# blasif/cocons

Measured on AMD Instinct MI355X. Metric: -2loglik evals/sec (dense cov_rns + Cholesky/solve/log-det, fp64) at n=10000, higher is better.
Workload: dtype f64

## Files before the change

cocons_amd/csrc/api.hip:

```cpp
#include <hip/hip_runtime.h>
#include <limits.h>
#include <math.h>
#include <stdarg.h>
#include <stdint.h>
#include <stdio.h>
#include <stdlib.h>
#include <string.h>
#include <unistd.h>
#include <time.h>
#include <dlfcn.h>
#include <rccl/rccl.h>

#include <algorithm>
#include <limits>
#include <memory>
#include <mutex>
#include <string>
#include <thread>
#include <vector>

#include "kernels.h"
#include "../../include/cocons_hip_diag.h"
#include "matern_device.hpp"

// ... 139 lines not shown
    bool fix = true;
    for (int i = 1; i < p; ++i)
        if (theta[TH_SMOOTH * p + i] != 0) fix = false;
    if (fix && smooth_limits[0] == smooth_limits[1]) {
        double v = smooth_limits[0];
        m.nu_fixed = v;
        m.smooth_kind = SMOOTH_ZERO;
        if (std::fabs(v - 0.5) < 1e-6) m.mode = MODE_HALF;
        else if (std::fabs(v - 1.5) < 1e-6) m.mode = MODE_THREEHALF;
        else if (std::fabs(v - 2.5) < 1e-6) m.mode = MODE_FIVEHALF;
        else m.mode = MODE_GEOM;
    } else {
        m.mode = MODE_GEOM;
        m.smooth_kind = SMOOTH_LOGISTIC_SQRT;
    }
    return m;
}

static LocArgs loc_args(int n, int p, const double *X, const double *locs, double *out, size_t stride, const ThetaVecs &tv,
                        int smooth_kind, const double *smooth_limits)
{
    LocArgs la;
    la.n = n; la.p = p;
    la.X = X; la.ldx = n;
    la.locs = locs; la.ldl = n;
    la.out = out; la.stride = stride;
    la.smooth_kind = smooth_kind;
    la.smooth_min = smooth_limits[0]; la.smooth_max = smooth_limits[1];
    la.th = tv;
    return la;
}

static inline int round_up(int v, int m) { return (v + m - 1) / m * m; }

struct RcclApi {
    void *h;
    ncclResult_t (*GetUniqueId)(ncclUniqueId *);
    ncclResult_t (*CommInitRank)(ncclComm_t *, int, ncclUniqueId, int);
    ncclResult_t (*CommInitAll)(ncclComm_t *, int, const int *);
    ncclResult_t (*CommDestroy)(ncclComm_t);
    ncclResult_t (*Broadcast)(const void *, void *, size_t, ncclDataType_t, int, ncclComm_t, hipStream_t);
    ncclResult_t (*AllReduce)(const void *, void *, size_t, ncclDataType_t, ncclRedOp_t, ncclComm_t, hipStream_t);
    ncclResult_t (*AllGather)(const void *, void *, size_t, ncclDataType_t, ncclComm_t, hipStream_t);
    ncclResult_t (*GroupStart)();
    ncclResult_t (*GroupEnd)();
    const char *(*GetErrorString)(ncclResult_t);
    ncclResult_t (*CommCount)(const ncclComm_t, int *);
    ncclResult_t (*CommUserRank)(const ncclComm_t, int *);
    ncclResult_t (*CommCuDevice)(const ncclComm_t, int *);
    ncclResult_t (*CommAbort)(ncclComm_t);
    ncclResult_t (*Send)(const void *, size_t, ncclDataType_t, int, ncclComm_t, hipStream_t);
    ncclResult_t (*Recv)(void *, size_t, ncclDataType_t, int, ncclComm_t, hipStream_t);
    ncclResult_t (*CommSplit)(ncclComm_t, int, int, ncclComm_t *, void *);
};

static RcclApi *rccl_api()
{
    static RcclApi api;
    static int state = 0;
    if (state == 0) {
        state = -1;
        std::vector<std::string> names;
        {
            Dl_info di;
            if (dladdr((void *)&hipGetDeviceCount, &di) && di.dli_fname) {
                std::string dir(di.dli_fname);
                size_t slash = dir.rfind('/');
                if (slash != std::string::npos) {
                    dir.resize(slash + 1);
                    names.push_back(dir + "librccl.so.1");
                    names.push_back(dir + "librccl.so");
                }
            }
        }
        names.push_back("librccl.so.1");
        names.push_back("librccl.so");
        names.push_back("/opt/rocm/lib/librccl.so.1");
        void *h = nullptr;
        for (const std::string &nm : names)
            if ((h = dlopen(nm.c_str(), RTLD_NOW | RTLD_LOCAL))) break;
        if (!h) { g_err = std::string("cannot load RCCL: ") + dlerror(); return nullptr; }
        api.h = h;
#define RSYM(field, name) *(void **)(&api.field) = dlsym(h, name); if (!api.field) { g_err = "RCCL symbol missing: " name; return nullptr; }
        RSYM(GetUniqueId, "ncclGetUniqueId")
        RSYM(CommInitRank, "ncclCommInitRank")
        RSYM(CommInitAll, "ncclCommInitAll")
        RSYM(CommDestroy, "ncclCommDestroy")
        RSYM(Broadcast, "ncclBroadcast")
        RSYM(AllReduce, "ncclAllReduce")
        RSYM(AllGather, "ncclAllGather")
        RSYM(GroupStart, "ncclGroupStart")
        RSYM(GroupEnd, "ncclGroupEnd")
        RSYM(GetErrorString, "ncclGetErrorString")
        RSYM(CommCount, "ncclCommCount")
        RSYM(CommUserRank, "ncclCommUserRank")
        RSYM(CommCuDevice, "ncclCommCuDevice")
        RSYM(CommAbort, "ncclCommAbort")
        RSYM(Send, "ncclSend")
        RSYM(Recv, "ncclRecv")
#undef RSYM
        *(void **)(&api.CommSplit) = dlsym(h, "ncclCommSplit");
        state = 1;
    }
    return state == 1 ? &api : nullptr;
}

static void rccl_comm_destroy(ncclComm_t c)
{
    RcclApi *R = rccl_api();
    if (R && c) R->CommDestroy(c);
}

#define NCCLCHK(expr)                                                             \
    do {                                                                          \
        ncclResult_t r__ = (expr);                                                \
        if (r__ != ncclSuccess) {                                                 \
            char b__[512];                                                        \
            snprintf(b__, sizeof b__, "%s failed: %s (%s:%d)", #expr,             \
                     rccl_api() ? rccl_api()->GetErrorString(r__) : "?", __FILE__, __LINE__); \
            g_err = b__;                                                          \
            return -200 - (int)r__;                                               \
        }                                                                         \
    } while (0)

struct cocons_fit {
    int n, p, r, q, device;
    pid_t pid;
    int npad, nt;
    int rhs_cap;
    int rhs_act;
    size_t lda;
    hipStream_t stream;
    bool own_stream;
    double *dX, *dlocs, *dz, *dxb;
    double *dloc;
    double *dA;
    double *dinv;
    int *dinfo;
    double *dout;
    double *hout;
    int *hinfo, *hinfo_init = nullptr;
    double smooth_limits[2];
    size_t out_cap;
    double *dlocp, *dXp, *dlocsp, *dstoch, *dquad, *dred;
    int pred_cap;
    int rank, world, nrhs_cur;
    int nslot;
    int n_user, pad0;
    double *xbuf[2];
    size_t xbuf_bytes;
    bool xbuf_own;
    hipEvent_t ev[8];
    hipStream_t stream2;
    hipEvent_t ev_eng;
    unsigned *dflags;
    int flags_cap;
    bool engine_ok;
    bool engine_live;
    bool engine_used;
    int border_clean = -1;
    int border_pending = -1;
    bool engine_active_last;
    int engine_skip;
    int engine_fails;
    int engine_retries;
    int engine_last_abort;
    long long engine_ops;
    double *dP; size_t dP_elems;
    double *dWt; int dWt_tiles;
    double *dpart;
    unsigned *ddag; size_t ddag_words;
    void *ddag_steps; int dag_nsteps; unsigned dag_ntasks;
    int dag_key[13];
    unsigned *ddag_ftab; size_t ddag_ftab_words;
    int dag_xcd_g;
    bool dag_have_ftab;
    size_t ddag_xcnt_off;
    unsigned long long *ddag_trace; size_t dag_trace_tasks;
    size_t dag_trace_elems;
    bool dag_next;
    int engine_pair_live;
    int engine_t0;
    size_t smb_off, smb_elems;
    size_t xmb_off, xmb_elems;
    double *dmbox; size_t dmbox_elems;
    bool follow_used, follow_off;
    double enq_host_us; long long enq_calls;
    bool dag_used;
    double dag_flops; int dag_events;
    int taper_nnz;
    int *d_tci, *d_trp;
    double *d_tval;
    std::vector<int> *taper_hi;
    int *d_thi; int taper_maxband;
    int skew;
    std::vector<int> *taper_inv;
    std::vector<int> *h_trp, *h_tci;
    std::vector<double> *h_tval;
    cocons_fit *taper_twin;
    std::vector<int> *twin_perm;
    float sim_ms[3];
    int coll_kind;
    int coll_rank, coll_world;
    ncclComm_t comm;
    bool comm_own;
    cocons_bcast_fn cb_bcast;
    cocons_allreduce_fn cb_allreduce;
    cocons_allgather_fn cb_allgather;
    struct ShardState *shard;
    void *cb_user;
    hipStream_t cstream;
    hipStream_t cstream_l;
    ncclComm_t comm_l;
    bool comm_l_own;
    double *dcoll;
    double upd_flops;
    std::vector<double> *h_locs, *h_X, *h_z, *h_xb;
    std::vector<cocons_fit *> *slots;
    bool sorted;
    cocons_fit *unsorted;
    std::recursive_mutex *op_mu;
    struct KrigeState *krige;
};

struct KrigeState {
    DevBuf<double> L;
    DevBuf<double> Q;
    DevBuf<double> w;
    DevBuf<double> loc;
    DevBuf<double> C;
    DevBuf<double> Xp, lp, locp;
    DevBuf<double> st, qd;
    std::vector<double> theta;
    int rows = 0;
    long long bytes = 0;
};

static void shard_state_free(struct ShardState *S);

static std::mutex g_reg_mutex;
static std::vector<cocons_fit *> g_registry;
static void registry_add(cocons_fit *f) { std::lock_guard<std::mutex> lk(g_reg_mutex); g_registry.push_back(f); }
static void registry_remove(cocons_fit *f)
{
    std::lock_guard<std::mutex> lk(g_reg_mutex);
    g_registry.erase(std::remove(g_registry.begin(), g_registry.end(), f), g_registry.end());
}

static int fit_check(cocons_fit *f)
{
    if (!f) return fail(-1, "null fit handle");
    if (f->pid != getpid())
        return fail(-2, "fit handle was created in another process (fork); create it in the worker");
    hipError_t e = hipSetDevice(f->device);
    if (e != hipSuccess) return fail(-3, "hipSetDevice: %s", hipGetErrorString(e));
    return 0;
}

#define FIT_ENTER(f)                                                   \
    if (int rc__ = fit_check(f)) return rc__;                          \
    std::lock_guard<std::recursive_mutex> op_guard__(*(f)->op_mu)

static int fit_alloc_matrix(cocons_fit *f, int rhs_rows)
{
    int cap = round_up(rhs_rows > 0 ? rhs_rows : 1, TILE);
    f->rhs_act = cap;
    f->border_clean = -1; f->border_pending = -1;
    if (f->dA && cap <= f->rhs_cap) return 0;
    if (f->dA) { HIPCHK(hipFree(f->dA)); f->dA = nullptr; }
    f->rhs_cap = cap;
    f->lda = (size_t)(f->skew > 0 ? f->skew * TILE : f->npad) + cap;
    HIPCHK(hipMalloc(&f->dA, f->lda * (size_t)f->npad * sizeof(double)));
    HIPCHK(hipMemsetAsync(f->dA, 0, f->lda * (size_t)f->npad * sizeof(double), f->stream));
    HIPCHK(hipStreamSynchronize(f->stream));
    return 0;
}

extern "C" void cocons_fit_destroy(cocons_fit *f)
{
    if (!f) return;
    registry_remove(f);
    if (f->op_mu) { f->op_mu->lock(); f->op_mu->unlock(); }
    if (f->pid == getpid()) {
        hipSetDevice(f->device);
        if (f->stream) hipStreamSynchronize(f->stream);
        if (f->stream2) hipStreamSynchronize(f->stream2);
        hipFree(f->dX); hipFree(f->dlocs); hipFree(f->dz); hipFree(f->dxb); hipFree(f->dloc);
        hipFree(f->dA); hipFree(f->dinv); hipFree(f->dinfo);
        hipFree(f->dlocp); hipFree(f->dXp); hipFree(f->dlocsp); hipFree(f->dstoch); hipFree(f->dquad); hipFree(f->dred);
        if (f->xbuf_own) { hipFree(f->xbuf[0]); hipFree(f->xbuf[1]); }
        hipHostFree(f->hinfo);
        for (auto &e : f->ev) if (e) hipEventDestroy(e);
        if (f->ev_eng) hipEventDestroy(f->ev_eng);
        hipFree(f->dflags);
        if (f->dmbox) hipFree(f->dmbox);
        hipFree(f->dP); hipFree(f->dWt); hipFree(f->ddag); hipFree(f->ddag_steps); hipFree(f->ddag_trace); hipFree(f->dpart);
        hipFree(f->ddag_ftab);
        hipFree(f->d_tci); hipFree(f->d_trp); hipFree(f->d_tval); hipFree(f->d_thi);
        if (f->cstream_l && f->cstream_l != f->cstream) { hipStreamSynchronize(f->cstream_l); hipStreamDestroy(f->cstream_l); }
        if (f->cstream) { hipStreamSynchronize(f->cstream); hipStreamDestroy(f->cstream); }
        shard_state_free(f->shard);
        hipFree(f->dcoll);
        if (f->comm_l && f->comm_l_own) rccl_comm_destroy(f->comm_l);
        if (f->comm && f->comm_own) rccl_comm_destroy(f->comm);
        if (f->slots) { for (auto c : *f->slots) cocons_fit_destroy(c); delete f->slots; f->slots = nullptr; }
        if (f->unsorted) { cocons_fit_destroy(f->unsorted); f->unsorted = nullptr; }
        if (f->taper_twin) { cocons_fit_destroy(f->taper_twin); f->taper_twin = nullptr; }
        delete f->krige; f->krige = nullptr;
        if (f->stream2) hipStreamDestroy(f->stream2);
        if (f->own_stream && f->stream) hipStreamDestroy(f->stream);
    }
    delete f->h_locs; delete f->h_X; delete f->h_z; delete f->h_xb;
    delete f->taper_hi; delete f->taper_inv;
    delete f->h_trp; delete f->h_tci; delete f->h_tval; delete f->twin_perm;
    delete f->op_mu;
    delete f;
}

static int engine_warm(cocons_fit *f);

static cocons_fit *fit_create_impl(int n, int p, int r, int q, const double *locs,
                                   const double *X, const double *z, const double *x_betas,
                                   const double *smooth_limits, int device, bool allow_sort, bool defer_matrix = false,
                                   bool want_engine = true, bool return_locked = false)
{
    if (n <= 0 || p <= 0 || p > COCONS_P_MAX || r < 0 || q < 0 || !locs || !X || !smooth_limits ||
        (r > 0 && !z) || (q > 0 && !x_betas)) {
        fail(-1, "cocons_fit_create: bad argument");
        return nullptr;
    }
    cocons_fit *f = new cocons_fit();
    memset(f, 0, sizeof *f);
    f->op_mu = new std::recursive_mutex();
    f->n = n; f->p = p; f->r = r; f->q = q;
    f->device = device < 0 ? 0 : device;
    f->pid = getpid();
    f->npad = round_up(n, TILE);
    f->nt = f->npad / TILE;
    f->smooth_limits[0] = smooth_limits[0];
    f->smooth_limits[1] = smooth_limits[1];
    f->world = 1;
#define CK(expr)                                                                  \
    do {                                                                          \
        hipError_t e__ = (expr);                                                  \
        if (e__ != hipSuccess) {                                                  \
            fail(-100, "cocons_fit_create: %s", hipGetErrorString(e__));          \
            cocons_fit_destroy(f);                                                \
            return nullptr;                                                       \
        }                                                                         \
    } while (0)
    CK(hipSetDevice(f->device));
    CK(hipStreamCreateWithFlags(&f->stream, hipStreamNonBlocking));
    f->own_stream = true;
    std::vector<int> perm(n);
    for (int i = 0; i < n; ++i) perm[i] = i;
    {
        const char *e = getenv("COCONS_SPATIAL_SORT");
        if (allow_sort && (e ? atoi(e) : 1) && n > 64) {
            double lo[2] = {locs[0], locs[n]}, hi[2] = {locs[0], locs[n]};
            for (int i = 0; i < n; ++i)
                for (int d = 0; d < 2; ++d) {
                    double v = locs[i + (size_t)d * n];
                    if (v < lo[d]) lo[d] = v;
                    if (v > hi[d]) hi[d] = v;
                }
            std::vector<unsigned long long> key(n);
            bool finite = true;
            for (int i = 0; i < n && finite; ++i) {
                unsigned q[2];
                for (int d = 0; d < 2; ++d) {
                    double span = hi[d] - lo[d];
                    double t = span > 0 ? (locs[i + (size_t)d * n] - lo[d]) / span : 0.0;
                    if (!(t >= 0.0 && t <= 1.0)) { finite = false; t = 0; }
                    q[d] = (unsigned)(t * 65535.0);
                }
                unsigned long long k = 0;
                for (int b = 0; b < 16; ++b)
                    k |= ((unsigned long long)((q[0] >> b) & 1u) << (2 * b)) | ((unsigned long long)((q[1] >> b) & 1u) << (2 * b + 1));
                key[i] = (k << 32) | (unsigned)i;
            }
            if (finite) {
                std::sort(key.begin(), key.end());
                auto path = [&](auto idx) {
                    double s = 0;
                    for (int i = 0; i + 1 < n; ++i) {
                        int a = idx(i), b = idx(i + 1);
                        double dx = locs[a] - locs[b], dy = locs[a + (size_t)n] - locs[b + (size_t)n];
                        s += std::sqrt(dx * dx + dy * dy);
                    }
                    return s;
                };
                double p_in = path([&](int i) { return i; });
                double p_mo = path([&](int i) { return (int)(key[i] & 0xffffffffu); });
                if (p_mo < 0.8 * p_in)
                    for (int i = 0; i < n; ++i) perm[i] = (int)(key[i] & 0xffffffffu);
            }
        }
    }
    f->h_locs = new std::vector<double>(locs, locs + (size_t)2 * n);
    f->h_X = new std::vector<double>(X, X + (size_t)n * p);
    f->h_z = new std::vector<double>();
    if (r > 0) f->h_z->assign(z, z + (size_t)n * r);
    f->h_xb = new std::vector<double>();
    if (q > 0) f->h_xb->assign(x_betas, x_betas + (size_t)n * q);
    f->sorted = false;
    for (int i = 0; i < n; ++i)
        if (perm[i] != i) { f->sorted = true; break; }
    f->n_user = n;
    {
        const char *e = getenv("COCONS_FRONT_PAD");
        f->pad0 = (allow_sort && (e ? atoi(e) : 1)) ? f->npad - n : 0;
        const char *e2 = getenv("COCONS_RHS_SLOTS");
        const int need = round_up(r + (q > p ? q : p) > 0 ? r + (q > p ? q : p) : 1, 16);
        f->nslot = (f->pad0 >= need && r > 0 && (e2 ? atoi(e2) : 1)) ? need : 0;
        f->pad0 -= f->nslot;
    }
    const int pad0 = f->pad0, nint = n + pad0;
    if (pad0 > 0) f->sorted = true;
    auto permute_pad = [&](const double *src, int ncol, bool zero_pad) {
        std::vector<double> out((size_t)nint * ncol);
        for (int c = 0; c < ncol; ++c) {
            for (int i = 0; i < pad0; ++i) out[(size_t)i + (size_t)c * nint] = zero_pad ? 0.0 : canon_nan(src[(size_t)perm[0] + (size_t)c * n]);
            for (int i = 0; i < n; ++i) out[(size_t)(pad0 + i) + (size_t)c * nint] = canon_nan(src[(size_t)perm[i] + (size_t)c * n]);
        }
        return out;
    };
    std::vector<double> plocs = permute_pad(locs, 2, false), pX = permute_pad(X, p, false), pz, pxb;
    if (r > 0) pz = permute_pad(z, r, true);
    if (q > 0) pxb = permute_pad(x_betas, q, true);
    locs = plocs.data(); X = pX.data();
    if (r > 0) z = pz.data();
    if (q > 0) x_betas = pxb.data();
    n = nint;
    f->n = n;
    CK(hipMalloc(&f->dX, (size_t)n * p * sizeof(double)));
    CK(hipMalloc(&f->dlocs, (size_t)n * 2 * sizeof(double)));
    CK(hipMemcpyAsync(f->dX, X, (size_t)n * p * sizeof(double), hipMemcpyHostToDevice, f->stream));
    CK(hipMemcpyAsync(f->dlocs, locs, (size_t)n * 2 * sizeof(double), hipMemcpyHostToDevice, f->stream));
    if (r > 0) {
        CK(hipMalloc(&f->dz, (size_t)n * r * sizeof(double)));
        CK(hipMemcpyAsync(f->dz, z, (size_t)n * r * sizeof(double), hipMemcpyHostToDevice, f->stream));
    }
    if (q > 0) {
        CK(hipMalloc(&f->dxb, (size_t)n * q * sizeof(double)));
        CK(hipMemcpyAsync(f->dxb, x_betas, (size_t)n * q * sizeof(double), hipMemcpyHostToDevice, f->stream));
    }
    CK(hipStreamSynchronize(f->stream));
    CK(hipMalloc(&f->dloc, (size_t)LOCP_FIELDS * f->npad * sizeof(double)));
    CK(hipMalloc(&f->dinv, 2 * 8 * 256 * sizeof(double)));
    int nr_max = r + (q > p ? q : p);
    f->out_cap = (size_t)(1 + nr_max * nr_max) * (size_t)(f->nt + 2);
    {
        double *dbase = nullptr, *hbase = nullptr;
        CK(hipMalloc(&dbase, (f->out_cap + 1) * sizeof(double)));
        CK(hipHostMalloc(&hbase, (f->out_cap + 2) * sizeof(double)));
        f->dinfo = (int *)dbase; f->dout = dbase + 1;
        f->hinfo = (int *)hbase; f->hout = hbase + 1;
        f->hinfo_init = (int *)(hbase + 1 + f->out_cap);
        f->hinfo_init[0] = 0x7f7f7f7f; f->hinfo_init[1] = 0;
    }
    for (auto &e : f->ev) CK(hipEventCreate(&e));
    f->engine_ok = want_engine;
// ... 258 lines not shown
    make_theta_vecs(theta, f->p, tv, true);
    ModeSel ms = select_mode(theta, f->p, f->smooth_limits, 0);
    launch_loc_params(loc_args(f->n, f->p, f->dX, f->dlocs, f->dloc, f->npad, tv, ms.smooth_kind, f->smooth_limits), f->stream);
    if (f->d_thi) launch_band_zero(f->dA, f->lda, f->d_thi, f->nt, f->taper_maxband, f->stream, f->skew);
    else HIPCHK(hipMemsetAsync(f->dA, 0, f->lda * (size_t)f->npad * sizeof(double), f->stream));
    launch_taper(ms.mode, false, f->n, f->taper_nnz, f->d_tci, f->d_trp, f->dloc, f->npad, f->dloc, f->npad,
                 ms.nu_fixed, nullptr, f->stream, f->d_tval, f->dA, f->lda, 0, f->skew, f->npad);
    launch_pad_identity(f->dA, f->lda, f->n, f->npad, f->stream, f->skew);
    return 0;
}

static int no_taper(cocons_fit *f, const char *who)
{
    if (f->taper_nnz > 0) return fail(-1, "%s: not available on a taper fit (cocons_neg2loglik_dense is)", who);
    return 0;
}

static void assemble_rhs(cocons_fit *f, const double *mean, bool use_trend, const double *xb, int nxb,
                         int col0, int col1, bool zero_rest = true, bool slots = false)
{
    if (slots) { zero_rest = false; col1 = f->n; }
    RhsArgs ra;
    memset(&ra, 0, sizeof ra);
    ra.n = f->n; ra.p = f->p; ra.X = f->dX; ra.ldx = f->n;
    ra.use_trend = use_trend ? 1 : 0;
    if (use_trend) for (int i = 0; i < f->p; ++i) ra.mean[i] = canon_nan(mean[i]);
    ra.src = f->dz; ra.lds = f->n;
    ra.out = f->dA; ra.ld = f->lda;
    ra.skew = f->skew; ra.npad = f->npad;
    ra.row0 = slots ? f->n : f->npad; ra.nrows = f->r;
    ra.nrows_zero = (nxb > 0 || !zero_rest) ? 0 : f->rhs_act - f->r;
    ra.col0 = col0; ra.ncols_out = col1;
    launch_rhs_rows(ra, f->stream);
    if (nxb > 0) {
        ra.use_trend = 0;
        ra.src = xb; ra.lds = f->n;
        ra.row0 = (slots ? f->n : f->npad) + f->r; ra.nrows = nxb;
        ra.nrows_zero = zero_rest ? f->rhs_act - f->r - nxb : 0;
        launch_rhs_rows(ra, f->stream);
    }
}

static void residual_row(cocons_fit *f, const double *mean, int z_col, double *out, size_t ld, int row0, int nrows_zero,
                         int ncols)
{
    RhsArgs ra;
    memset(&ra, 0, sizeof ra);
    ra.n = f->n; ra.p = f->p; ra.X = f->dX; ra.ldx = f->n; ra.use_trend = 1;
    for (int i = 0; i < f->p; ++i) ra.mean[i] = canon_nan(mean[i]);
    ra.src = f->dz + (size_t)z_col * f->n; ra.lds = f->n;
    ra.out = out; ra.ld = ld; ra.row0 = row0; ra.nrows = 1; ra.nrows_zero = nrows_zero;
    ra.col0 = 0; ra.ncols_out = ncols;
    ra.skew = f->skew; ra.npad = f->npad;
    launch_rhs_rows(ra, f->stream);
}

static void clear_border(cocons_fit *f)
{
    RhsArgs ra;
    memset(&ra, 0, sizeof ra);
    ra.n = f->n; ra.p = f->p; ra.X = f->dX; ra.ldx = f->n; ra.src = f->dX; ra.lds = f->n;
    ra.out = f->dA; ra.ld = f->lda; ra.row0 = f->npad; ra.nrows = 0; ra.nrows_zero = f->rhs_act;
    ra.col0 = 0; ra.ncols_out = f->npad;
    ra.skew = f->skew; ra.npad = f->npad;
    launch_rhs_rows(ra, f->stream);
}

static std::vector<double> host_trend(const cocons_fit *f, const double *mean)
{
    const int n = f->n;
    std::vector<double> tr(n, 0.0);
    for (int j = 0; j < f->p; ++j)
        for (int i = 0; i < n; ++i) tr[i] += (*f->h_X)[(size_t)i + (size_t)j * n] * mean[j];
    return tr;
}

struct FactorView {
    double *A;
    size_t lda;
    int nt, mt;
    const int *hi = nullptr;
    int skew = 0;
    int trim = 0;
    bool dag_ok = false;
};

static FactorView main_view(cocons_fit *f)
{
    FactorView v;
    v.A = f->dA; v.lda = f->lda; v.nt = f->nt; v.mt = f->nt + f->rhs_act / TILE;
    v.hi = (f->taper_hi && !f->taper_hi->empty()) ? f->taper_hi->data() : nullptr;
    v.skew = f->skew;
    return v;
}

static int band_hi(const FactorView &v, int k)
{
    if (!v.hi) return -1;
    int h = v.hi[k];
    if (k + 1 < v.nt && v.hi[k + 1] > h) h = v.hi[k + 1];
    const int need = k + 4 < v.nt ? k + 4 : v.nt;
    if (h < need) h = need;
    return h < v.nt ? h : v.nt;
}

static bool follow_on(cocons_fit *f);
static void potrf_solve(cocons_fit *f, double *A, size_t lda, int tile, int r0, int r1, double *q, hipStream_t s, int br, int er)
{
    if (follow_on(f) && ((size_t)tile + 1) * ENGINE_MBOX_DOUBLES <= f->smb_off) {
        f->follow_used = true;
        launch_potrf_follow(A, lda, tile * TILE, r0, r1, q, f->dinfo,
                            f->dmbox + (size_t)tile * ENGINE_MBOX_DOUBLES, (unsigned *)(f->dinfo + 1), s, br, er);
        return;
    }
    launch_potrf_tile(A, lda, tile * TILE, q, f->dinfo, s);
    launch_trsm_tile(A, lda, tile * TILE, r0, r1, q, s, nullptr, nullptr, br, er);
}

static void panel_ops(cocons_fit *f, const FactorView &v, int k, hipStream_t s)
{
    const int nt = v.nt, mt = v.mt;
    double *A = v.A;
    const size_t lda = v.lda;
    double *q0 = f->dinv, *q1 = f->dinv + 8 * 256;
    const int hb = band_hi(v, k);
    const int br = hb >= 0 ? hb * TILE : -1, er = nt * TILE;
    const int r1 = mt * TILE - 64 * v.trim;
    potrf_solve(f, A, lda, k, (k + 1) * TILE, r1, q0, s, br, er);
    if (k + 1 < nt) {
        launch_update(A, lda, k * TILE, TILE, k + 1, mt, k + 1, k + 2, true, s, nullptr, -1, nullptr, nullptr, nullptr, hb, nt,
                      0, v.trim);
        potrf_solve(f, A, lda, k + 1, (k + 2) * TILE, r1, q1, s, br, er);
    }
}

struct Tunables {
    int engine = 1;
    int upd_dynamic = 1;
    int dag = 1;
    int dag_lead = 1600, dag_lead2 = 600, dag_lead3 = 1800;
    int dag_min_tiles = 2000;
    int dag_split = 1;
    int dag_xcd = 1;
    int dag_order = 1, dag_bw = 16, dag_bh = 16;
    int dag_xcd_min_quota = 128;
    int dag_xcc_quota = -1;
    int engine_block0 = 1;
    int engine_pair = 1;
    int panel_fused = 1;
    int panel_follow = 1;
    int panel_split = 32;
    int panel_diag = 1;
    int potrf_follow = 1;
    int dag_trace = 0;
    int gate_sabotage = 0;
    int host_delay_us = 0, host_delay_tile = -1, engine_in_wait_ms = 0;
    bool init = false;
};
static Tunables &tun()
{
    static Tunables t;
    if (!t.init) {
        auto rd = [](const char *name, int &v) { const char *e = getenv(name); if (e) v = atoi(e); };
        rd("COCONS_ENGINE", t.engine);
        rd("COCONS_UPD_DYNAMIC", t.upd_dynamic);
        rd("COCONS_DAG", t.dag);
        rd("COCONS_DAG_LEAD", t.dag_lead);
        rd("COCONS_DAG_LEAD2", t.dag_lead2);
        rd("COCONS_DAG_LEAD3", t.dag_lead3);
        rd("COCONS_DAG_MIN_TILES", t.dag_min_tiles);
        rd("COCONS_DAG_SPLIT", t.dag_split);
        rd("COCONS_DAG_XCC_QUOTA", t.dag_xcc_quota);
        rd("COCONS_DAG_XCD", t.dag_xcd);
        rd("COCONS_DAG_ORDER", t.dag_order);
        rd("COCONS_DAG_BW", t.dag_bw);
        rd("COCONS_DAG_BH", t.dag_bh);
        rd("COCONS_ENGINE_PAIR", t.engine_pair);
        rd("COCONS_ENGINE_BLOCK0", t.engine_block0);
        rd("COCONS_PANEL_FUSED", t.panel_fused);
        rd("COCONS_POTRF_FOLLOW", t.potrf_follow);
        rd("COCONS_PANEL_FOLLOW", t.panel_follow);
        rd("COCONS_PANEL_DIAG", t.panel_diag);
        rd("COCONS_PANEL_SPLIT", t.panel_split);
        rd("COCONS_DEBUG_HOST_DELAY_US", t.host_delay_us);
        rd("COCONS_DEBUG_HOST_DELAY_TILE", t.host_delay_tile);
        t.init = true;
    }
    return t;
}

static bool follow_on(cocons_fit *f)
{
    return tun().potrf_follow != 0 && !f->follow_off && f->dmbox != nullptr &&
           f->smb_off >= ((size_t)f->nt + 2) * ENGINE_MBOX_DOUBLES;
}

extern "C" int cocons_debug_tune(const char *name, int value)
{
    if (!name) return fail(-1, "cocons_debug_tune: null name");
    Tunables &t = tun();
    std::string k(name);
    if (k == "engine") t.engine = value;
    else if (k == "upd_dynamic") t.upd_dynamic = value;
    else if (k == "dag") t.dag = value;
    else if (k == "dag_lead") t.dag_lead = value;
    else if (k == "dag_lead2") t.dag_lead2 = value;
    else if (k == "dag_lead3") t.dag_lead3 = value;
    else if (k == "dag_min_tiles") t.dag_min_tiles = value;
    else if (k == "dag_split") t.dag_split = value;
    else if (k == "dag_xcc_quota") t.dag_xcc_quota = value;
    else if (k == "dag_xcd") t.dag_xcd = value;
    else if (k == "dag_order") t.dag_order = value;
    else if (k == "dag_xcd_min_quota") t.dag_xcd_min_quota = value;
    else if (k == "dag_bw") t.dag_bw = value < 1 ? 1 : value;
    else if (k == "dag_bh") t.dag_bh = value < 1 ? 1 : value;
    else if (k == "dag_trace") t.dag_trace = value;
    else if (k == "engine_pair") t.engine_pair = value;
    else if (k == "engine_block0") t.engine_block0 = value;
    else if (k == "panel_fused") t.panel_fused = value;
    else if (k == "potrf_follow") t.potrf_follow = value;
    else if (k == "panel_follow") t.panel_follow = value;
    else if (k == "panel_diag") t.panel_diag = value;
    else if (k == "panel_split") t.panel_split = value;
    else if (k == "gate_sabotage") t.gate_sabotage = value;
    else if (k == "host_delay_us") t.host_delay_us = value;
    else if (k == "host_delay_tile") t.host_delay_tile = value;
    else if (k == "engine_in_wait_ms") t.engine_in_wait_ms = value;
    else if (k == "upd_waves") set_update_waves(value);
    else if (k == "w8_max_tiles") set_update_w8_max_tiles(value);
    else if (k == "c_wt") set_update_c_wt(value);
    else return fail(-1, "cocons_debug_tune: unknown switch %s", name);
    return 0;
}

static int device_cus()
{
    int dev = 0, cus = 256;
    (void)hipGetDevice(&dev);
    (void)hipDeviceGetAttribute(&cus, hipDeviceAttributeMultiprocessorCount, dev);
    return cus;
}

static int dag_xcc_quota()
{
    if (tun().dag_xcc_quota >= 0) return tun().dag_xcc_quota;
    static int derived = -1;
    if (derived < 0) {
        int dev = 0, cus = 256;
        (void)hipGetDevice(&dev);
        (void)hipDeviceGetAttribute(&cus, hipDeviceAttributeMultiprocessorCount, dev);
        const int xcds = 8;
        const int cpx = cus % xcds == 0 ? cus / xcds : 32;
        derived = (cpx - 1) * 7 - 9;
        if (derived < 8) derived = 8;
    }
    return derived;
}

static bool engine_enabled() { return tun().engine != 0; }

static void timed_update(cocons_fit *f, const FactorView &v, int k, int kw, int t0, int t1, hipStream_t s,
                         std::vector<hipEvent_t> *ev_upd, unsigned *sig, int sig_tile, unsigned *queue = nullptr,
                         int skip_tiles = 0)
{
    const int mt = v.mt;
    if (t1 <= t0) return;
    const int hb = band_hi(v, k);
    if (hb >= 0 && hb < t1) t1 = hb;
    if (t1 <= t0) return;
    unsigned *abort_word = sig ? (unsigned *)(f->dinfo + 1) : nullptr;
    hipEvent_t a = nullptr, b = nullptr;
    if (ev_upd) {
        hipEventCreate(&a); hipEventCreate(&b);
        hipEventRecord(a, s);
    }
    const int kskip = (k == 0 && !v.hi) ? (f->pad0 / 16) * 16 : 0;
    launch_update(v.A, v.lda, k * TILE + kskip, kw * TILE - kskip, t0, mt, t0, t1, true, s, sig, sig_tile, nullptr,
                  abort_word, queue, hb, v.nt, 0, v.trim, skip_tiles > 0 ? 2 * t0 : 0, skip_tiles > 0 ? 2 * (t0 + skip_tiles) : 0);
    if (ev_upd) {
        hipEventRecord(b, s);
        ev_upd->push_back(a); ev_upd->push_back(b);
    }
}

static void count_update_flops(cocons_fit *f, int kw, int t0)
{
    double m = (double)f->n_user - ((double)t0 * TILE - (double)f->pad0);
    if (m > (double)f->n_user) m = (double)f->n_user;
    if (m < 0) m = 0;
    const double K = (double)kw * TILE - (t0 == kw ? (double)f->pad0 : 0.0);
    f->upd_flops += K * m * (m + 1.0) + 2.0 * K * (double)f->nrhs_cur * m;
}

static bool engine_wanted(cocons_fit *f, const FactorView &v)
{
    return engine_enabled() && f->engine_ok && f->stream2 != nullptr && f->engine_skip == 0 && v.nt > 4;
}

static int flags_reset(cocons_fit *f, int nt)
{
    if (f->flags_cap < nt) {
        if (f->stream2) HIPCHK(hipStreamSynchronize(f->stream2));
        if (f->dflags) { HIPCHK(hipFree(f->dflags)); f->dflags = nullptr; }
        f->flags_cap = round_up(nt + 8, 64);
        HIPCHK(hipMalloc(&f->dflags, (4 * (size_t)f->flags_cap + 64) * sizeof(unsigned)));
    }
    HIPCHK(hipMemsetAsync(f->dflags, 0, (4 * (size_t)f->flags_cap + 64) * sizeof(unsigned), f->stream));
    return 0;
}

static int mbox_reset(cocons_fit *f, int nt, bool engine_schedule = true)
{
    const size_t tiles = ((size_t)nt + 2) * ENGINE_MBOX_DOUBLES;
    const bool panel = tun().panel_follow && tun().panel_fused && tun().engine_pair;
    const size_t smb = panel && tun().panel_diag ? ((size_t)nt / 2 + 2) * PANEL_SMBOX_DOUBLES : 0;
    const size_t xmb = panel && tun().panel_split ? (2 * ((size_t)nt + 2) + 4) * PANEL_XMBOX_DOUBLES : 0;
    const size_t need = tiles + smb + xmb;
    if (f->dmbox_elems < need) {
        HIPCHK(hipStreamSynchronize(f->stream));
        if (f->stream2) HIPCHK(hipStreamSynchronize(f->stream2));
        if (f->dmbox) { HIPCHK(hipFree(f->dmbox)); f->dmbox = nullptr; f->dmbox_elems = 0; }
        HIPCHK(hipMalloc(&f->dmbox, need * sizeof(double)));
        f->dmbox_elems = need;
    }
    f->smb_off = tiles; f->smb_elems = smb;
    f->xmb_off = tiles + smb; f->xmb_elems = xmb;
    HIPCHK(hipMemsetAsync(f->dmbox, 0xff, (engine_schedule ? need : tiles) * sizeof(double), f->stream));
    return 0;
}

static unsigned *tile_queue(cocons_fit *f, int k)
{
    const int dyn = tun().upd_dynamic;
    return dyn ? f->dflags + 3 * (size_t)f->flags_cap + 64 + k / 2 : nullptr;
}

static int engine_warm(cocons_fit *f)
{
    if (!engine_enabled() || f->nt <= 4 || !f->engine_ok) { f->engine_ok = f->engine_ok && f->stream2 != nullptr; return 0; }
    if (!f->stream2) HIPCHK(hipStreamCreateWithFlags(&f->stream2, hipStreamNonBlocking));
    if (int rc = flags_reset(f, f->nt)) return rc;
    HIPCHK(hipStreamSynchronize(f->stream));
    {
        std::vector<hipStream_t> losers;
        int ok = 0;
        for (int attempt = 0; attempt < 8; ++attempt) {
            ok = streams_run_concurrently(f->stream2, f->stream, f->dflags + 3 * (size_t)f->flags_cap + 8);
            if (ok != 0) break;
            losers.push_back(f->stream2);
            f->stream2 = nullptr;
            if (hipStreamCreateWithFlags(&f->stream2, hipStreamNonBlocking) != hipSuccess) { ok = -1; break; }
        }
        unsigned *words = f->dflags + 3 * (size_t)f->flags_cap + 8;
        for (int round = 0; ok == 1 && round < 8; ++round) {
            std::vector<cocons_fit *> others;
            {
                std::lock_guard<std::mutex> lk(g_reg_mutex);
                for (size_t i = g_registry.size(); i-- > 0 && others.size() < 4;) {
                    cocons_fit *o = g_registry[i];
                    if (o == f || o->pid != f->pid || o->device != f->device || !o->own_stream || !o->stream || !o->stream2 ||
                        !o->engine_ok || !o->op_mu->try_lock())
                        continue;
                    if (hipStreamQuery(o->stream) == hipSuccess && hipStreamQuery(o->stream2) == hipSuccess) others.push_back(o);
                    else o->op_mu->unlock();
                }
            }
            (void)hipGetLastError();
            int clash = 0;
            for (cocons_fit *o : others) {
                int a = streams_run_concurrently(f->stream2, o->stream, words);
                if (a < 0) { ok = -1; break; }
                if (a == 0) { clash = 1; break; }
                if (f->own_stream) {
                    int b = streams_run_concurrently(o->stream2, f->stream, words);
                    if (b < 0) { ok = -1; break; }
                    if (b == 0) { clash = 2; break; }
                }
            }
            for (cocons_fit *o : others) o->op_mu->unlock();
            if (ok != 1 || clash == 0) break;
            hipStream_t &mine = clash == 1 ? f->stream2 : f->stream;
            losers.push_back(mine);
            mine = nullptr;
            if (hipStreamCreateWithFlags(&mine, hipStreamNonBlocking) != hipSuccess) { ok = -1; break; }
            int again = streams_run_concurrently(f->stream2, f->stream, words);
            if (again < 0) { ok = -1; break; }
            if (again == 0) {
                hipStream_t &other = clash == 1 ? f->stream2 : f->stream;
                (void)other;
                bool fixed = false;
                for (int t2 = 0; t2 < 4 && !fixed; ++t2) {
                    losers.push_back(mine);
                    mine = nullptr;
                    if (hipStreamCreateWithFlags(&mine, hipStreamNonBlocking) != hipSuccess) { ok = -1; break; }
                    const int r2 = streams_run_concurrently(f->stream2, f->stream, words);
                    if (r2 < 0) { ok = -1; break; }
                    fixed = r2 == 1;
                }
                if (ok != 1) break;
                if (!fixed) { ok = 0; break; }
            }
        }
        for (hipStream_t l : losers) hipStreamDestroy(l);
        if (ok < 0) { (void)hipGetLastError(); return fail(-100, "engine_warm: stream self-test failed"); }
        if (ok == 0) { f->engine_ok = false; return 0; }
        HIPCHK(hipMemsetAsync(f->dflags, 0, (4 * (size_t)f->flags_cap + 64) * sizeof(unsigned), f->stream));
        HIPCHK(hipStreamSynchronize(f->stream));
    }
    launch_potrf_engine(nullptr, 0, 0, 0, f->dinv, f->dinfo, f->dflags, f->dflags, f->dflags, (unsigned *)(f->dinfo + 1),
                        f->dflags + 3 * (size_t)f->flags_cap, f->stream2);
    if (tun().dag)
        launch_potrf_engine(nullptr, 0, 0, 0, f->dinv, f->dinfo, f->dflags, f->dflags, f->dflags, (unsigned *)(f->dinfo + 1),
                            f->dflags + 3 * (size_t)f->flags_cap, f->stream2, f->dinv, f->dinv, 0);
    HIPCHK(hipGetLastError());
    if (f->stream2) HIPCHK(hipStreamSynchronize(f->stream2));
    return 0;
}

static bool dag_wanted(cocons_fit *f, const FactorView &v)
{
    return tun().dag != 0 && v.dag_ok && !v.hi && !v.skew && v.nt > 4 && f->world == 1;
}

static int dag_prepare(cocons_fit *f, const FactorView &v)
{
    const size_t elems = v.lda * (size_t)f->npad;
    if (f->dP_elems != elems) {
        HIPCHK(hipStreamSynchronize(f->stream));
        if (f->stream2) HIPCHK(hipStreamSynchronize(f->stream2));
        if (f->dP) { HIPCHK(hipFree(f->dP)); f->dP = nullptr; f->dP_elems = 0; }
        HIPCHK(hipMalloc(&f->dP, elems * sizeof(double)));
        HIPCHK(hipMemsetAsync(f->dP, 0, elems * sizeof(double), f->stream));
        f->dP_elems = elems;
    }
    if (!f->dpart) HIPCHK(hipMalloc(&f->dpart, (size_t)2 * 16 * 64 * 64 * sizeof(double)));
    if (f->dWt_tiles < v.nt) {
        HIPCHK(hipStreamSynchronize(f->stream));
        if (f->stream2) HIPCHK(hipStreamSynchronize(f->stream2));
        if (f->dWt) { HIPCHK(hipFree(f->dWt)); f->dWt = nullptr; }
        HIPCHK(hipMalloc(&f->dWt, (size_t)v.nt * TILE * TILE * sizeof(double)));
        HIPCHK(hipMemsetAsync(f->dWt, 0, (size_t)v.nt * TILE * TILE * sizeof(double), f->stream));
        f->dWt_tiles = v.nt;
    }
    const int kskip = (f->pad0 / 16) * 16;
    const int q_all = dag_xcc_quota();
    const int xcd_g = (tun().dag_xcd && device_cus() == 256 && (q_all == 0 || q_all >= tun().dag_xcd_min_quota)) ? 5 : 0;
    const int key[13] = {v.nt, v.mt, v.trim, kskip, tun().dag_lead, tun().dag_min_tiles, tun().dag_split, tun().dag_lead2, tun().dag_lead3,
                         tun().dag_order, xcd_g, tun().dag_bw, tun().dag_bh};
    if (memcmp(key, f->dag_key, sizeof key) != 0 || !f->ddag_steps) {
        std::vector<DagStepHost> steps;
        std::vector<unsigned> ftab;
        const bool want_tab = tun().dag_order != 0 || xcd_g > 0;
        const unsigned ntasks = dag_build_steps(v.nt, v.mt, v.trim, kskip, tun().dag_lead, tun().dag_min_tiles, tun().dag_split, steps,
                                                tun().dag_lead2, tun().dag_lead3, want_tab ? &ftab : nullptr, xcd_g,
                                                tun().dag_order ? tun().dag_bw : 0, tun().dag_bh);
        HIPCHK(hipStreamSynchronize(f->stream));
        if (f->stream2) HIPCHK(hipStreamSynchronize(f->stream2));
        if (f->ddag_steps) { HIPCHK(hipFree(f->ddag_steps)); f->ddag_steps = nullptr; }
        HIPCHK(hipMalloc(&f->ddag_steps, (steps.size() + 1) * sizeof(DagStepHost)));
        HIPCHK(hipMemcpyAsync(f->ddag_steps, steps.data(), steps.size() * sizeof(DagStepHost), hipMemcpyHostToDevice, f->stream));
        if (f->ddag_ftab_words < ftab.size()) {
            if (f->ddag_ftab) { HIPCHK(hipFree(f->ddag_ftab)); f->ddag_ftab = nullptr; f->ddag_ftab_words = 0; }
            HIPCHK(hipMalloc(&f->ddag_ftab, ftab.size() * sizeof(unsigned)));
            f->ddag_ftab_words = ftab.size();
        }
        if (!ftab.empty())
            HIPCHK(hipMemcpyAsync(f->ddag_ftab, ftab.data(), ftab.size() * sizeof(unsigned), hipMemcpyHostToDevice, f->stream));
        f->dag_xcd_g = want_tab ? xcd_g : 0;
        f->dag_have_ftab = want_tab && !ftab.empty();
        HIPCHK(hipStreamSynchronize(f->stream));
        f->dag_nsteps = (int)steps.size(); f->dag_ntasks = ntasks;
        memcpy(f->dag_key, key, sizeof key);
        const size_t T64 = 2 * (size_t)v.mt;
        size_t words = 64 + T64 * (T64 + 1) / 2 + (steps.size() + 2) * T64 + steps.size() + 64 + 16 * (steps.size() + 2);
        words = (words + 31) / 32 * 32;
        f->ddag_xcnt_off = words;
        words += 8 * 32;
        if (f->ddag_words < words) {
            if (f->ddag) { HIPCHK(hipFree(f->ddag)); f->ddag = nullptr; }
            HIPCHK(hipMalloc(&f->ddag, words * sizeof(unsigned)));
            f->ddag_words = words;
        }
    }
    HIPCHK(hipMemsetAsync(f->ddag, 0, f->ddag_words * sizeof(unsigned), f->stream));
    const size_t trace_elems = (size_t)f->dag_ntasks * 5 + 8 * (size_t)(v.nt + 2);
    if (tun().dag_trace && f->dag_trace_elems < trace_elems) {
        HIPCHK(hipStreamSynchronize(f->stream));
        if (f->stream2) HIPCHK(hipStreamSynchronize(f->stream2));
        if (f->ddag_trace) { HIPCHK(hipFree(f->ddag_trace)); f->ddag_trace = nullptr; f->dag_trace_elems = 0; }
        HIPCHK(hipMalloc(&f->ddag_trace, trace_elems * sizeof(unsigned long long)));
        f->dag_trace_elems = trace_elems;
    }
    f->dag_trace_tasks = (tun().dag_trace && f->ddag_trace) ? f->dag_ntasks : 0;
    if (f->dag_trace_tasks)
        HIPCHK(hipMemsetAsync(f->ddag_trace, 0, trace_elems * sizeof(unsigned long long), f->stream));
    return 0;
}

extern "C" long long cocons_debug_dag_trace(cocons_fit *f, int *nsteps_out, int *steps_out, unsigned long long *stamps_out,
                                            unsigned long long *engine_out)
{
    FIT_ENTER(f);
    if (!f->ddag_steps) return fail(-1, "cocons_debug_dag_trace: no DAG factorisation on this handle yet");
    if (nsteps_out) *nsteps_out = f->dag_nsteps;
    HIPCHK(hipStreamSynchronize(f->stream));
    if (steps_out)
        HIPCHK(hipMemcpyAsync(steps_out, f->ddag_steps, (size_t)f->dag_nsteps * sizeof(DagStepHost), hipMemcpyDeviceToHost, f->stream));
    if (stamps_out) {
        if (!f->ddag_trace || f->dag_trace_tasks != f->dag_ntasks)
            return fail(-1, "cocons_debug_dag_trace: tracing was off (cocons_debug_tune(\"dag_trace\", 1))");
        HIPCHK(hipMemcpyAsync(stamps_out, f->ddag_trace, (size_t)f->dag_ntasks * 4 * sizeof(unsigned long long), hipMemcpyDeviceToHost,
                              f->stream));
        if (engine_out)
            HIPCHK(hipMemcpyAsync(engine_out, f->ddag_trace + 4 * (size_t)f->dag_ntasks, 8 * (size_t)(f->nt + 2) * sizeof(unsigned long long),
                                  hipMemcpyDeviceToHost, f->stream));
    }
    HIPCHK(hipStreamSynchronize(f->stream));
    return (long long)f->dag_ntasks;
}

extern "C" int cocons_debug_dag_words(cocons_fit *f, int count, unsigned *out)
{
    FIT_ENTER(f);
    if (!f->ddag || !out || count < 1 || (size_t)count > f->ddag_words) return fail(-1, "cocons_debug_dag_words: bad argument or no DAG factorisation yet");
    HIPCHK(hipStreamSynchronize(f->stream));
    HIPCHK(hipMemcpyAsync(out, f->ddag, (size_t)count * sizeof(unsigned), hipMemcpyDeviceToHost, f->stream));
    HIPCHK(hipStreamSynchronize(f->stream));
    return 0;
}

static int engine_start(cocons_fit *f, const FactorView &v)
{
    if (f->engine_live) return 0;
    const int nt = v.nt;
    hipStream_t M = f->stream;
    if (int rc = flags_reset(f, nt)) return rc;
    unsigned *in = f->dflags, *out = f->dflags + f->flags_cap, *xr = f->dflags + 2 * (size_t)f->flags_cap;
    f->dag_next = dag_wanted(f, v);
    if (f->dag_next) {
        if (int rc = dag_prepare(f, v)) return rc;
        if (f->dag_nsteps < 2) f->dag_next = false;
    }
    f->engine_pair_live = tun().engine_pair != 0 ? 1 : 0;
    if (f->engine_pair_live || (tun().potrf_follow && !f->follow_off))
        if (int rc = mbox_reset(f, nt > f->nt ? nt : f->nt)) return rc;
    HIPCHK(hipEventRecord(f->ev_eng, M));
    HIPCHK(hipStreamWaitEvent(f->stream2, f->ev_eng, 0));
    unsigned *alive_w = f->dflags + 3 * (size_t)f->flags_cap;
    f->engine_t0 = (tun().engine_block0 && !v.hi) ? 0 : 2;
    launch_potrf_engine(v.A, v.lda, f->engine_t0, nt, f->dinv, f->dinfo, in, out, xr, (unsigned *)(f->dinfo + 1),
                        alive_w, f->stream2, f->dag_next ? f->dWt : nullptr,
                        f->dag_next ? f->dP : nullptr, f->dag_next ? 2 * f->dag_nsteps : 0,
                        (f->dag_next && f->dag_trace_tasks) ? f->ddag_trace + 4 * (size_t)f->dag_ntasks : nullptr,
                        f->engine_pair_live ? f->dmbox : nullptr, tun().engine_in_wait_ms);
    f->engine_live = true;
    return 0;
}

static int factorize(cocons_fit *f, const FactorView &v, std::vector<hipEvent_t> *ev_upd)
{
    const int nt = v.nt, mt = v.mt;
    hipStream_t M = f->stream;
    launch_front_identity(v.A, v.lda, f->pad0, mt * TILE, M);
    f->follow_used = false;
    if (!engine_wanted(f, v)) {
        f->engine_used = false;
        f->dag_used = false;
        if (int rc = flags_reset(f, nt)) return rc;
        if (tun().potrf_follow && !f->follow_off)
            if (int rc = mbox_reset(f, nt > f->nt ? nt : f->nt, false)) return rc;
        if (v.hi) {
            for (int k = 0; k < nt; ++k) {
                const int hb = v.hi[k] < nt ? v.hi[k] : nt;
                double *q = f->dinv + (size_t)(k & 1) * 2048;
                double *Ak = band_base(v.A, k, v.skew);
                const int e0 = v.skew ? k + v.skew : nt, e1 = e0 + (mt - nt);
                potrf_solve(f, Ak, v.lda, k, (k + 1) * TILE, e1 * TILE - 64 * v.trim, q, M, hb * TILE, e0 * TILE);
                if (k + 1 < nt)
                    launch_update(v.A, v.lda, k * TILE, TILE, k + 1, mt, k + 1, hb < nt ? hb : nt, true, M, nullptr, -1,
                                  nullptr, nullptr, nullptr, hb, nt, v.skew, v.trim);
            }
            return 0;
        }
        for (int k = 0; k < nt; k += 2) {
            panel_ops(f, v, k, M);
            if (k + 2 < nt) {
                if (ev_upd) count_update_flops(f, 2, k + 2);
                timed_update(f, v, k, 2, k + 2, nt, M, ev_upd, nullptr, -1, tile_queue(f, k));
            }
        }
        return 0;
    }
    if (int rc = engine_start(f, v)) return rc;
    f->engine_live = false;
    f->engine_used = true;
    unsigned *in = f->dflags, *out = f->dflags + f->flags_cap, *xr = f->dflags + 2 * (size_t)f->flags_cap;
    unsigned *abort_word = (unsigned *)(f->dinfo + 1);
    unsigned *alive = f->dflags + 3 * (size_t)f->flags_cap;
    if (tun().gate_sabotage > 0) { --tun().gate_sabotage; alive += 1; }
    const bool block0 = f->engine_t0 == 0;
    launch_engine_gate(alive, abort_word, M, false, f->engine_ops++ == 0,
                       f->engine_pair_live,
                       (block0 && tun().gate_sabotage == 0 && alive == f->dflags + 3 * (size_t)f->flags_cap) ? in : nullptr);
    const int rend = mt * TILE - 64 * v.trim;
    auto panel_for = [&](int t, bool allow_diag) -> int {
        const bool two = t + 1 < nt;
        const int r0 = two ? t + 2 : t + 1;
        const int hb = band_hi(v, t);
        const int br = hb >= 0 ? hb * TILE : -1, er = nt * TILE;
        if (two && hb < 0 && tun().panel_fused) {
            const bool fol = f->engine_pair_live && tun().panel_follow && f->dmbox != nullptr;
            const int next_tiles = t + 2 < nt ? (t + 3 < nt ? 2 : 1) : 0;
            const bool dg = allow_diag && fol && tun().panel_diag && next_tiles > 0 &&
                            ((size_t)(t >> 1) + 1) * PANEL_SMBOX_DOUBLES <= f->smb_elems;
            const int nstrips = (rend - r0 * TILE) / 64;
            const bool sp = fol && tun().panel_split > 0 && nstrips >= tun().panel_split &&
                            (size_t)nstrips * PANEL_XMBOX_DOUBLES <= f->xmb_elems;
            launch_panel_pair(v.A, v.lda, t * TILE, r0 * TILE, rend, f->dinv + (size_t)(t & 1) * 2048,
                              f->dinv + (size_t)((t + 1) & 1) * 2048, out + t, xr + t, out + t + 1, abort_word, M,
                              fol ? f->dmbox + (size_t)t * ENGINE_MBOX_DOUBLES : nullptr,
                              fol ? f->dmbox + (size_t)(t + 1) * ENGINE_MBOX_DOUBLES : nullptr,
                              dg ? f->dmbox + f->smb_off + (size_t)(t >> 1) * PANEL_SMBOX_DOUBLES : nullptr,
                              dg ? (next_tiles == 2 ? 10 : 3) : 0, in, t + 2, sp ? f->dmbox + f->xmb_off : nullptr);
            return (dg && nstrips >= (next_tiles == 2 ? 4 : 2)) ? next_tiles : 0;
        }
        launch_trsm_tile(v.A, v.lda, t * TILE, r0 * TILE, rend, f->dinv + (size_t)(t & 1) * 2048, M,
                         out + t, abort_word, br, er);
        if (two) {
            launch_update(v.A, v.lda, t * TILE, TILE, r0, mt, t + 1, t + 2, false, M, nullptr, -1, xr + t, abort_word,
                          nullptr, hb, nt, 0, v.trim);
            launch_trsm_tile(v.A, v.lda, (t + 1) * TILE, r0 * TILE, rend,
                             f->dinv + (size_t)((t + 1) & 1) * 2048, M, out + t + 1, abort_word, br, er);
        }
        return 0;
    };
    int diag_done = 0;
    if (block0) diag_done = panel_for(0, !f->dag_next);
    else panel_ops(f, v, 0, M);
    f->dag_used = f->dag_next;
    int k_first = 0;
    if (f->dag_next) {
        const size_t T64 = 2 * (size_t)mt;
        unsigned *queue = f->ddag, *tdone = f->ddag + 64, *pdone = tdone + T64 * (T64 + 1) / 2;
        unsigned *pall = pdone + ((size_t)f->dag_nsteps + 2) * T64;
        unsigned *dcount = pall + (size_t)f->dag_nsteps + 64;
        hipEvent_t ea = nullptr, eb = nullptr;
        if (ev_upd) {
            const double before = f->upd_flops;
            for (int s = 0; s < f->dag_nsteps; ++s) count_update_flops(f, 2, 2 * s + 2);
            f->dag_flops = f->upd_flops - before;
            hipEventCreate(&ea); hipEventCreate(&eb);
            hipEventRecord(ea, M);
        }
        launch_dag(v.A, v.lda, f->dP, f->dWt, (const DagStepHost *)f->ddag_steps, f->dag_nsteps, f->dag_ntasks, queue, tdone,
                   pdone, (int)T64, pall, f->dpart, dcount, in, out, xr, abort_word, M, f->dag_trace_tasks ? f->ddag_trace : nullptr,
                   alive, dag_xcc_quota(), f->dag_trace_tasks ? (unsigned *)(f->ddag_trace + 4 * (size_t)f->dag_ntasks + 8 * (size_t)(v.nt + 2)) : nullptr,
                   f->dag_have_ftab ? f->ddag_ftab : nullptr, f->dag_xcd_g, f->ddag + f->ddag_xcnt_off);
        if (ev_upd) { hipEventRecord(eb, M); ev_upd->push_back(ea); ev_upd->push_back(eb); f->dag_events = 1; }
        k_first = 2 * f->dag_nsteps;
    }
    for (int k = k_first > 0 ? k_first - 2 : 0; k + 2 < nt; k += 2) {
        const int t = k + 2;
        if (tun().host_delay_us > 0 && t + 2 == tun().host_delay_tile) usleep((useconds_t)tun().host_delay_us);
        if (k >= k_first) {
            if (ev_upd) count_update_flops(f, 2, t);
            timed_update(f, v, k, 2, t, nt, M, ev_upd, in, t, tile_queue(f, k), diag_done);
        }
        diag_done = panel_for(t, k + 4 < nt);
    }
    if (mt == nt) launch_engine_gate(out + (nt - 1), abort_word, M, true);
    return 0;
}

static int reset_info(cocons_fit *f)
{
    HIPCHK(hipMemcpyAsync(f->dinfo, f->hinfo_init, 2 * sizeof(int), hipMemcpyHostToDevice, f->stream));
    return 0;
}

static int enqueue_eval_impl(cocons_fit *f, const double *theta, const double *mean, bool use_trend,
                             const double *xb, int nxb, std::vector<hipEvent_t> *ev_upd, bool stage_events);
static int enqueue_eval(cocons_fit *f, const double *theta, const double *mean, bool use_trend,
                        const double *xb, int nxb, std::vector<hipEvent_t> *ev_upd, bool stage_events)
{
    struct timespec t0, t1;
    clock_gettime(CLOCK_MONOTONIC, &t0);
    const int rc = enqueue_eval_impl(f, theta, mean, use_trend, xb, nxb, ev_upd, stage_events);
    clock_gettime(CLOCK_MONOTONIC, &t1);
    f->enq_host_us += (t1.tv_sec - t0.tv_sec) * 1e6 + (t1.tv_nsec - t0.tv_nsec) * 1e-3;
    f->enq_calls++;
    return rc;
}

extern "C" int cocons_debug_host_enqueue(cocons_fit *f, double *out)
{
    if (!f || !out) return fail(-1, "cocons_debug_host_enqueue: null argument");
    double us = f->enq_host_us; long long n = f->enq_calls;
    if (f->slots) for (cocons_fit *c : *f->slots) { us += c->enq_host_us; n += c->enq_calls; }
    out[0] = n ? us / (double)n : 0.0; out[1] = (double)n;
    return 0;
}

static int enqueue_eval_impl(cocons_fit *f, const double *theta, const double *mean, bool use_trend,
                             const double *xb, int nxb, std::vector<hipEvent_t> *ev_upd, bool stage_events)
{
    const int nrhs = f->r + nxb;
    f->nrhs_cur = nrhs;
    const int was_clean = f->border_clean;
    const double *was_A = f->dA;
    if (int rc = fit_alloc_matrix(f, nrhs)) return rc;
    const bool zero_rest = !(was_clean == nrhs && was_A == f->dA);
    f->border_pending = nrhs;
    if (stage_events) hipEventRecord(f->ev[0], f->stream);
    if (int rc = reset_info(f)) return rc;
    if (f->taper_nnz > 0) { if (int rc = assemble_sigma_taper(f, theta)) return rc; }
    else assemble_sigma(f, theta, 0, 0, f->npad);
    const bool slots = f->nslot >= nrhs && f->nslot > 0;
    FactorView fv = main_view(f);
    if (slots) fv.mt = fv.nt;
    else fv.trim = (f->rhs_act - nrhs >= 64) ? 1 : 0;
    fv.dag_ok = true;
    if (engine_wanted(f, fv))
        if (int rc = engine_start(f, fv)) return rc;
    assemble_rhs(f, mean, use_trend, xb, nxb, 0, f->npad, zero_rest, slots);
    if (stage_events) hipEventRecord(f->ev[1], f->stream);
    if (int rc = factorize(f, fv, ev_upd)) return rc;
    if (stage_events) hipEventRecord(f->ev[2], f->stream);
    launch_finalize(f->dA, f->lda, f->n, slots ? f->n : f->npad, nrhs, f->dout, f->stream, f->skew, f->npad,
                    f->dag_used ? f->dP : nullptr, f->dag_used ? 2 * TILE * f->dag_nsteps : 0);
    HIPCHK(hipMemcpyAsync(f->hinfo, f->dinfo, (size_t)(2 + nrhs * nrhs) * sizeof(double),
                          hipMemcpyDeviceToHost, f->stream));
    if (stage_events) hipEventRecord(f->ev[3], f->stream);
    HIPCHK(hipGetLastError());
    return 0;
}

static void debug_abort_report(cocons_fit *f)
{
    fprintf(stderr, "cocons: hand-off time-out, code 0x%x\n", f->hinfo[1]);
    const unsigned cls = abort_class((unsigned)f->hinfo[1]);
    if (!f->dag_used || !f->ddag || cls < ABORT_DAG_FIRST || cls > ABORT_DAG_LAST) return;
    unsigned rec[7] = {0, 0, 0, 0, 0, 0, 0}, now = 0, qn = 0;
    hipMemcpyAsync(rec, f->ddag + 8, sizeof rec, hipMemcpyDeviceToHost, f->stream);
    hipStreamSynchronize(f->stream);
    if (rec[2] < f->ddag_words) hipMemcpyAsync(&now, f->ddag + rec[2], sizeof now, hipMemcpyDeviceToHost, f->stream);
    hipMemcpyAsync(&qn, f->ddag, sizeof qn, hipMemcpyDeviceToHost, f->stream);
    hipStreamSynchronize(f->stream);
    fprintf(stderr, "cocons: DAG wait: task %u (of %u, counter now %u) code 0x%x waited for word %u >= %u, saw %u, holds %u now; "
            "%.1f ms, %u polls\n", rec[0], f->dag_ntasks, qn, rec[1], rec[2], rec[3], rec[4], now, rec[5] * 1e-5, rec[6]);
    if (const char *dump = getenv("COCONS_DEBUG_ABORT_DUMP")) {
        static int ndump = 0;
        char path[512];
        snprintf(path, sizeof path, "%s.%d", dump, ndump++);
        if (FILE *fp = fopen(path, "wb")) {
            const unsigned ntr = f->dag_trace_tasks ? 1u : 0u;
            unsigned hdr[16] = {0xDA6D0001u, (unsigned)f->nt, (unsigned)f->dag_nsteps, f->dag_ntasks, (unsigned)f->ddag_words,
                                (unsigned)f->flags_cap, ntr, (unsigned)f->hinfo[1], qn, now, 0, 0, 0, 0, 0, 0};
            fwrite(hdr, sizeof hdr, 1, fp);
            fwrite(rec, sizeof rec, 1, fp);
            std::vector<DagStepHost> sh((size_t)f->dag_nsteps);
            hipMemcpyAsync(sh.data(), f->ddag_steps, sh.size() * sizeof(DagStepHost), hipMemcpyDeviceToHost, f->stream);
            std::vector<unsigned> w((size_t)f->ddag_words), fl(4 * (size_t)f->flags_cap + 64);
            hipMemcpyAsync(w.data(), f->ddag, w.size() * sizeof(unsigned), hipMemcpyDeviceToHost, f->stream);
            hipMemcpyAsync(fl.data(), f->dflags, fl.size() * sizeof(unsigned), hipMemcpyDeviceToHost, f->stream);
            hipStreamSynchronize(f->stream);
            fwrite(sh.data(), sizeof(DagStepHost), sh.size(), fp);
            fwrite(w.data(), sizeof(unsigned), w.size(), fp);
            fwrite(fl.data(), sizeof(unsigned), fl.size(), fp);
            if (ntr) {
                std::vector<unsigned long long> st((size_t)f->dag_ntasks * 5 + 8 * (size_t)(f->nt + 2));
                hipMemcpyAsync(st.data(), f->ddag_trace, st.size() * sizeof(unsigned long long), hipMemcpyDeviceToHost, f->stream);
                hipStreamSynchronize(f->stream);
                fwrite(st.data(), sizeof(unsigned long long), st.size(), fp);
            }
            fclose(fp);
            fprintf(stderr, "cocons: state written to %s\n", path);
        }
    }
    if (f->dag_trace_tasks && !getenv("COCONS_DEBUG_ABORT_DUMP")) {
        std::vector<unsigned long long> st((size_t)f->dag_ntasks * 4);
        hipMemcpyAsync(st.data(), f->ddag_trace, st.size() * sizeof(unsigned long long), hipMemcpyDeviceToHost, f->stream);
        hipStreamSynchronize(f->stream);
        unsigned long long tmin = ~0ull;
        for (size_t i = 0; i < st.size(); i += 4) if (st[i] && st[i] < tmin) tmin = st[i];
        int shown = 0;
        for (unsigned L = 0; L < f->dag_ntasks && shown < 40; ++L) {
            const unsigned long long *q = &st[(size_t)L * 4];
            if (q[0] && !q[3]) {
                fprintf(stderr, "   unfinished task %u: drawn %.1f us, inputs %s, product %s\n", L, (q[0] - tmin) * 0.01,
                        q[1] ? "complete" : "WAITING", q[2] ? "done" : "-");
                ++shown;
            }
        }
    }
}

static int info_status(cocons_fit *f)
{
    if (f->hinfo[1] != 0) {
        if (getenv("COCONS_DEBUG_ABORT")) debug_abort_report(f);
        return fail(ENGINE_ABORT, "hand-off between the diagonal-tile engine and the main stream timed out");
    }
    f->engine_active_last = f->engine_used;
    if (f->engine_used) f->engine_fails = 0;
    else if (f->engine_skip > 0) --f->engine_skip;
    int info = f->hinfo[0];
    if (info != 0x7f7f7f7f) {
        info -= f->pad0;
        if (info < 1) info = 1;
        if (info > f->n_user) info = f->n_user;
        g_err = "leading minor not positive";
        return info;
    }
    f->border_clean = f->border_pending;
    f->border_pending = -1;
    return 0;
}

static bool engine_retry(cocons_fit *f, int st)
{
    if (st != ENGINE_ABORT || !(f->engine_used || f->follow_used)) return false;
    f->engine_retries++;
    f->engine_last_abort = f->hinfo[1];
    if (!f->engine_used || abort_class((unsigned)f->hinfo[1]) == ABORT_FOLLOW) f->follow_off = true;
    if (f->engine_fails < 6) f->engine_fails++;
    f->engine_skip = 1 << f->engine_fails;
    f->engine_live = false;
    f->engine_used = false;
    if (f->stream2) hipStreamSynchronize(f->stream2);
    return true;
}

static int run_eval(cocons_fit *f, const double *theta, const double *mean, bool use_trend, const double *xb, int nxb)
{
    for (;;) {
        if (int rc = enqueue_eval(f, theta, mean, use_trend, xb, nxb, nullptr, false)) return rc;
        HIPCHK(hipStreamSynchronize(f->stream));
        const int st = info_status(f);
        if (!engine_retry(f, st)) return st;
    }
}

template <class F> static int run_op(cocons_fit *f, const char *who, F &&enqueue)
{
    for (;;) {
        if (int rc = reset_info(f)) return rc;
        if (int rc = enqueue()) return rc;
        HIPCHK_AT(who, hipMemcpyAsync(f->hinfo, f->dinfo, 2 * sizeof(int), hipMemcpyDeviceToHost, f->stream));
        HIPCHK_AT(who, hipGetLastError());
        HIPCHK_AT(who, hipStreamSynchronize(f->stream));
        const int st = info_status(f);
        if (!engine_retry(f, st)) return st;
    }
}

extern "C" int cocons_fit_engine_state(cocons_fit *f, int *out)
{
    if (!f || !out) return fail(-1, "cocons_fit_engine_state: null argument");
    out[0] = f->engine_active_last ? 1 : 0;
    out[1] = f->engine_retries;
    out[2] = f->engine_last_abort;
    if (f->slots)
        for (cocons_fit *c : *f->slots) {
            out[1] += c->engine_retries;
            if (!out[2]) out[2] = c->engine_last_abort;
        }
    for (cocons_fit *c : {f->taper_twin, f->unsorted})
        if (c) {
            out[1] += c->engine_retries;
            if (!out[2]) out[2] = c->engine_last_abort;
        }
    return 0;
}

static const double LOG_2PI = 1.8378770664093454835606594728112;
static void dense_collect(cocons_fit *f, double *sum_logliks, double *parts);
static int sharded_eval(cocons_fit *f, const double *theta, const double *mean, double *sum_logliks, double *parts);

extern "C" int cocons_neg2loglik_dense(cocons_fit *f, const double *theta, const double *mean,
                                       double *sum_logliks, double *parts)
{
    FIT_ENTER(f);
    if (!theta || !mean || !sum_logliks) return fail(-1, "cocons_neg2loglik_dense: null argument");
    if (f->r < 1) return fail(-1, "cocons_neg2loglik_dense: fit has no z");
    if (f->coll_kind < 0) return fail(-7, "cocons_neg2loglik_dense: the communicator of this fit was aborted after an error");
    if (f->coll_kind) return sharded_eval(f, theta, mean, sum_logliks, parts);
    if (int st = run_eval(f, theta, mean, true, nullptr, 0)) return st;
    dense_collect(f, sum_logliks, parts);
    return 0;
}

static void dense_collect(cocons_fit *f, double *sum_logliks, double *parts)
{
    const int nr = f->r;
    double logdet = f->hout[0], total = 0.0;
    for (int k = 0; k < nr; ++k) {
        double quad = f->hout[1 + k * nr + k];
        total += f->n_user * LOG_2PI + 2 * logdet + quad;
        if (parts) parts[1 + k] = quad;
    }
    if (parts) parts[0] = logdet;
    *sum_logliks = total;
}

static void slot_stream_apart(cocons_fit *f, cocons_fit *c)
{
    if (!c->own_stream || !c->dflags) return;
    unsigned *words = c->dflags + 3 * (size_t)c->flags_cap + 8;
    std::vector<hipStream_t> losers;
    for (int attempt = 0; attempt < 8; ++attempt) {
        bool clash = false;
        std::vector<cocons_fit *> peers{f};
        if (f->slots) for (cocons_fit *o : *f->slots) if (o != c) peers.push_back(o);
        for (cocons_fit *o : peers) {
            if (hipStreamQuery(o->stream) != hipSuccess) { (void)hipGetLastError(); continue; }
            const int r = streams_run_concurrently(o->stream, c->stream, words);
            if (r == 0) { clash = true; break; }
            if (r < 0) { (void)hipGetLastError(); break; }
        }
        if (!clash) break;
        losers.push_back(c->stream);
        c->stream = nullptr;
        if (hipStreamCreateWithFlags(&c->stream, hipStreamNonBlocking) != hipSuccess) { c->stream = losers.back(); losers.pop_back(); break; }
    }
    for (hipStream_t l : losers) hipStreamDestroy(l);
    if (c->stream2 && streams_run_concurrently(c->stream2, c->stream, words) == 0) c->engine_ok = false;
    (void)hipMemsetAsync(c->dflags, 0, (4 * (size_t)c->flags_cap + 64) * sizeof(unsigned), c->stream);
    (void)hipStreamSynchronize(c->stream);
}

static cocons_fit *clone_for_slot(cocons_fit *f, bool want_engine)
{
    if (f->taper_nnz <= 0) {
        cocons_fit *c = fit_create_impl(f->n_user, f->p, f->r, 0, f->h_locs->data(), f->h_X->data(), f->h_z->data(), nullptr,
                                        f->smooth_limits, f->device, true, false, want_engine, true);
        if (c) {
            if (!c->dflags && flags_reset(c, c->nt) != 0) { c->op_mu->unlock(); cocons_fit_destroy(c); return nullptr; }
            hipStreamSynchronize(c->stream);
            slot_stream_apart(f, c);
            c->engine_ok = c->engine_ok && c->stream2 != nullptr;
            c->op_mu->unlock();
        }
        return c;
    }
    cocons_fit *c = fit_create_impl(f->n_user, f->p, f->r, 0, f->h_locs->data(), f->h_X->data(), f->h_z->data(), nullptr,
                                    f->smooth_limits, f->device, false, true, false, true);
    if (!c) return nullptr;
    struct Unlock { cocons_fit *c; ~Unlock() { if (c) c->op_mu->unlock(); } } unlock{c};
    auto drop = [&]() { unlock.c = nullptr; c->op_mu->unlock(); cocons_fit_destroy(c); return (cocons_fit *)nullptr; };
    if (!c->dflags && flags_reset(c, c->nt) != 0) return drop();
    hipStreamSynchronize(c->stream);
    slot_stream_apart(f, c);
    c->skew = f->skew;
    if (fit_alloc_matrix(c, f->r + f->p) != 0) return drop();
    const size_t nnz = (size_t)f->taper_nnz;
    bool ok = hipMalloc(&c->d_tci, nnz * sizeof(int)) == hipSuccess &&
              hipMalloc(&c->d_trp, (size_t)(f->n + 1) * sizeof(int)) == hipSuccess &&
              hipMalloc(&c->d_tval, nnz * sizeof(double)) == hipSuccess &&
              hipMemcpyAsync(c->d_tci, f->d_tci, nnz * sizeof(int), hipMemcpyDeviceToDevice, c->stream) == hipSuccess &&
              hipMemcpyAsync(c->d_trp, f->d_trp, (size_t)(f->n + 1) * sizeof(int), hipMemcpyDeviceToDevice, c->stream) == hipSuccess &&
              hipMemcpyAsync(c->d_tval, f->d_tval, nnz * sizeof(double), hipMemcpyDeviceToDevice, c->stream) == hipSuccess;
    c->taper_hi = new std::vector<int>(*f->taper_hi);
    c->taper_inv = new std::vector<int>(*f->taper_inv);
    c->taper_maxband = f->taper_maxband;
    if (ok && f->d_thi)
        ok = hipMalloc(&c->d_thi, (size_t)f->nt * sizeof(int)) == hipSuccess &&
             hipMemcpyAsync(c->d_thi, f->d_thi, (size_t)f->nt * sizeof(int), hipMemcpyDeviceToDevice, c->stream) == hipSuccess;
    if (ok) ok = hipStreamSynchronize(c->stream) == hipSuccess;
    if (!ok) return drop();
    c->taper_nnz = f->taper_nnz;
    c->engine_ok = f->engine_ok && c->stream2 != nullptr;
    return c;
}

extern "C" int cocons_neg2loglik_batch(cocons_fit *f, int nb, const double *thetas, const double *means,
                                       double *values, int *status)
{
    FIT_ENTER(f);
    if (nb < 0 || (nb > 0 && (!thetas || !means || !values || !status)))
        return fail(-1, "cocons_neg2loglik_batch: bad argument");
    if (f->r < 1) return fail(-1, "cocons_neg2loglik_batch: fit has no z");
    static int nslots_env = -1, batch_engine = -2;
    if (nslots_env < 0) {
        const char *e = getenv("COCONS_BATCH_SLOTS");
        nslots_env = e ? atoi(e) : 0;
        if (nslots_env < 0) nslots_env = 0;
        if (nslots_env > 8) nslots_env = 8;
        const char *e2 = getenv("COCONS_BATCH_ENGINE");
        batch_engine = e2 ? (atoi(e2) ? 1 : 0) : -1;
    }
    const bool eng_mode = batch_engine >= 0 ? batch_engine == 1 : false;
    const int nslots = nslots_env > 0 ? nslots_env : (eng_mode ? 2 : 4);
    int S = nb < nslots ? (nb > 0 ? nb : 1) : nslots;
    if (!f->slots) f->slots = new std::vector<cocons_fit *>();
    std::vector<std::unique_lock<std::recursive_mutex>> slot_locks;
    for (cocons_fit *c : *f->slots) slot_locks.emplace_back(*c->op_mu);
    while ((int)f->slots->size() < S - 1) {
        cocons_fit *c = clone_for_slot(f, eng_mode);
        if (!c) { (void)hipGetLastError(); break; }
        slot_locks.emplace_back(*c->op_mu);
        f->slots->push_back(c);
    }
    const bool engine_saved = f->engine_ok;
    if (!eng_mode) {
        if (S > 1) f->engine_ok = false;
        for (auto c : *f->slots) c->engine_ok = false;
    }
    if (S > (int)f->slots->size() + 1) S = (int)f->slots->size() + 1;
    for (int i = 0; i < nb; ++i) { values[i] = NAN; status[i] = -1; }
    std::vector<int> pending(S, -1);
    const int tp = 6 * f->p;
    int rc_all = 0;
    auto slot_of = [&](int s) { return s == 0 ? f : (*f->slots)[s - 1]; };
    auto collect = [&](int s) -> int {
        cocons_fit *c = slot_of(s);
        int i = pending[s];
        if (i < 0) return 0;
        pending[s] = -1;
        HIPCHK(hipStreamSynchronize(c->stream));
        int st = info_status(c);
        if (engine_retry(c, st)) {
            if (int rc = enqueue_eval(c, thetas + (size_t)i * tp, means + (size_t)i * f->p, true, nullptr, 0, nullptr, false))
                return rc;
            HIPCHK(hipStreamSynchronize(c->stream));
            st = info_status(c);
        }
        status[i] = st;
        if (st == 0) dense_collect(c, &values[i], nullptr);
        else values[i] = NAN;
        return 0;
    };
    for (int i = 0; i < nb; ++i) {
        int s = i % S;
        if (int rc = collect(s)) { rc_all = rc; break; }
        cocons_fit *c = slot_of(s);
        if (int rc = enqueue_eval(c, thetas + (size_t)i * tp, means + (size_t)i * f->p, true, nullptr, 0, nullptr, false)) {
            rc_all = rc;
            break;
        }
        pending[s] = i;
    }
    for (int s = 0; s < S; ++s)
        if (int rc = collect(s)) rc_all = rc_all ? rc_all : rc;
    f->engine_ok = engine_saved;
    return rc_all;
}

static int host_spd_solve(int q, std::vector<double> &W, int nb, std::vector<double> &B, double *logdet_half)
{
    double ld = 0;
    for (int j = 0; j < q; ++j) {
        double d = W[j + j * q];
        for (int k = 0; k < j; ++k) d -= W[j + k * q] * W[j + k * q];
        if (!(d > 0)) return j + 1;
        d = std::sqrt(d);
        W[j + j * q] = d;
        ld += std::log(d);
        for (int i = j + 1; i < q; ++i) {
            double s = W[i + j * q];
            for (int k = 0; k < j; ++k) s -= W[i + k * q] * W[j + k * q];
            W[i + j * q] = s / d;
        }
    }
    for (int c = 0; c < nb; ++c) {
        double *b = &B[(size_t)c * q];
        for (int i = 0; i < q; ++i) {
            double s = b[i];
            for (int k = 0; k < i; ++k) s -= W[i + k * q] * b[k];
            b[i] = s / W[i + i * q];
        }
        for (int i = q - 1; i >= 0; --i) {
            double s = b[i];
            for (int k = i + 1; k < q; ++k) s -= W[k + i * q] * b[k];
            b[i] = s / W[i + i * q];
        }
    }
    *logdet_half = ld;
    return 0;
}

// ... 1596 lines not shown
```

cocons_amd/csrc/chol.hip:

```cpp
#include <hip/hip_runtime.h>
#include <limits.h>
#include <stdlib.h>
#include <string.h>
#include <algorithm>
#include <atomic>
#include <vector>
#include "kernels.h"

namespace cocons {

typedef double d4 __attribute__((ext_vector_type(4)));

#define MFMA64(a, b, c) __builtin_amdgcn_mfma_f64_16x16x4f64((a), (b), (c), 0, 0, 0)
#define MFMA64_NEGA(a, b, c) __builtin_amdgcn_mfma_f64_16x16x4f64((a), (b), (c), 0, 0, 1)

__device__ __forceinline__ void blk_mma(d4 &acc, const d4 &P, const d4 &Q)
{
    acc = MFMA64(Q[0], P[0], acc);
    acc = MFMA64(Q[1], P[1], acc);
    acc = MFMA64(Q[2], P[2], acc);
    acc = MFMA64(Q[3], P[3], acc);
}

__device__ __forceinline__ d4 lds_blk(const double *blk, int lane)
// ... 715 lines not shown
#pragma unroll
                for (int r = 0; r < 4; ++r)
                    B[j][r] = load_wt((const double *)((const char *)Sb + (lo + (unsigned)(16 * j + 4 * r) * ldab)));
#pragma unroll
            for (int j = 0; j < 8; ++j) {
                d4 L = lds_blk(smem + (j * (j + 1) / 2 + j) * 256, lane);
                double Q[4];
#pragma unroll
                for (int s = 0; s < 4; ++s) Q[s] = QALL[j * 256 + s * 64 + lane];
                trsm16(B[j], L, Q);
                d4 NX = -B[j];
#pragma unroll
                for (int jj = j + 1; jj < 8; ++jj) {
                    d4 Lb = lds_blk(smem + (jj * (jj + 1) / 2 + j) * 256, lane);
                    blk_mma(B[jj], NX, Lb);
                }
            }
            asm volatile("" : "+v"(lo));
#pragma unroll
            for (int j = 0; j < 8; ++j)
#pragma unroll
                for (int r = 0; r < 4; ++r)
                    store_wt((double *)((char *)const_cast<double *>(Sb) + (lo + (unsigned)(16 * j + 4 * r) * ldab)), B[j][r]);
            if (dag_blk) {
                double *Pb = e.pbuf + (size_t)(c1 + 16 * wave) + (size_t)c0 * lda;
                asm volatile("" : "+v"(lo));
#pragma unroll
                for (int j = 0; j < 8; ++j)
#pragma unroll
                    for (int r = 0; r < 4; ++r)
                        store_wt((double *)((char *)Pb + (lo + (unsigned)(16 * j + 4 * r) * ldab)), B[j][r]);
            }
            __syncthreads();
#pragma unroll
            for (int j = 0; j < 8; ++j) lds_blk_store(XS + (wave * 8 + j) * 256, lane, B[j]);
        }
        asm volatile("s_waitcnt vmcnt(0)" ::: "memory");
        __syncthreads();
        if (tid == 0) signal_add(e.xr + t);
        if (tr && tid == 0) tr[4] = __builtin_amdgcn_s_memrealtime();
        {
            d4 cur = glb_blk_wt(A, lda, c1 + 16 * c_tri_ib[wave], c1 + 16 * (wave - c_tri_ib[wave] * (c_tri_ib[wave] + 1) / 2), lane);
            for (int bb = wave; bb < 36; bb += 8) {
                const int ib = c_tri_ib[bb], kb = bb - ib * (ib + 1) / 2;
                d4 nxt = cur;
                if (bb + 8 < 36) {
                    const int ib2 = c_tri_ib[bb + 8], kb2 = bb + 8 - ib2 * (ib2 + 1) / 2;
                    nxt = glb_blk_wt(A, lda, c1 + 16 * ib2, c1 + 16 * kb2, lane);
                }
                d4 acc = cur;
#pragma unroll
                for (int j = 0; j < 8; ++j) {
                    d4 P = lds_blk(XS + (ib * 8 + j) * 256, lane);
                    d4 Qk = lds_blk(XS + (kb * 8 + j) * 256, lane);
                    P = -P;
                    blk_mma(acc, P, Qk);
                }
                glb_blk_store_wt(A, lda, c1 + 16 * ib, c1 + 16 * kb, lane, acc);
                cur = nxt;
            }
        }
        asm volatile("s_waitcnt vmcnt(0)" ::: "memory");
        __syncthreads();
        if (tr && tid == 0) tr[5] = __builtin_amdgcn_s_memrealtime();
        potrf_tile_body<true>(A, lda, c1, e.dinv + (size_t)((t + 1) & 1) * 2048, e.info, smem, dag_blk ? QALL : nullptr,
                              dag_blk ? e.wbuf + (size_t)(t + 1) * TILE * TILE : nullptr, XI);
        if (tr && tid == 0) tr[6] = __builtin_amdgcn_s_memrealtime();
        asm volatile("s_waitcnt vmcnt(0)" ::: "memory");
        __syncthreads();
        if (tid == 0) signal_add(e.out + t + 1);
        if (tr && tid == 0) tr[7] = __builtin_amdgcn_s_memrealtime();
    }
}

__global__ void __launch_bounds__(512)
potrf_follow_kernel(double *A, size_t lda, int c0, double *q_out, int *info, double *mbox, int r0, int nb1, int e0, int nstrips,
                    unsigned *abort_word)
{
    extern __shared__ double smem[];
    if (blockIdx.x == 0) {
        potrf_tile_body<false>(A, lda, c0, q_out, info, smem, nullptr, nullptr, nullptr, mbox);
        return;
    }
    double *LST = smem;
    int *okp = (int *)(smem + 18 * 256);
    const int tid = threadIdx.x, lane = tid & 63;
    const int wave = __builtin_amdgcn_readfirstlane(tid >> 6);
    const int half = __builtin_amdgcn_readfirstlane(tid >> 8);
    const int strip = 2 * ((int)blockIdx.x - 1) + half;
    const bool valid = strip < nstrips;
    const int rs = (strip < nb1 ? r0 + 64 * strip : e0 + 64 * (strip - nb1)) + 16 * (wave & 3);
    const double *mb = mbox;
    d4 B[8];
#pragma unroll
    for (int j = 0; j < 8; ++j) B[j] = valid ? glb_blk(A, lda, rs, c0 + 16 * j, lane) : (d4){0.0, 0.0, 0.0, 0.0};
    if (tid == 0) *okp = 1;
    __syncthreads();
    double v[5];
    MBOX_FETCH(0)
#pragma unroll
    for (int j = 0; j < 8; ++j) {
        double *LS = LST + (j & 1) * (9 * 256);
        MBOX_COMPLETE(j, abort_word, abort_code(ABORT_FOLLOW, (unsigned)(c0 / TILE)))
#pragma unroll
        for (int i = 0; i < 5; ++i)
            if (half + 2 * i <= 8 - j) LS[tid + 512 * i] = v[i];
        __syncthreads();
        if (*okp == 0) return;
        if (j < 7) MBOX_FETCH(j + 1)
        int ln = lane;
        asm volatile("" : "+v"(ln));
        d4 L = lds_blk(LS, ln);
        double Q[4];
#pragma unroll
        for (int s = 0; s < 4; ++s) Q[s] = LS[(8 - j) * 256 + s * 64 + ln];
        trsm16(B[j], L, Q);
        d4 NX = -B[j];
#pragma unroll
        for (int jj = j + 1; jj < 8; ++jj) {
            d4 Lb = lds_blk(LS + (jj - j) * 256, ln);
            blk_mma(B[jj], NX, Lb);
        }
    }
    if (valid) {
#pragma unroll
        for (int j = 0; j < 8; ++j) glb_blk_store(A, lda, rs, c0 + 16 * j, lane, B[j]);
    }
}

template <bool WT>
__device__ __forceinline__ void fetch_factor_tile(const double *A, size_t lda, int c0, const double *qin, double *SL, double *QS, int tid)
{
    const int i = tid & 15, k = tid >> 4;
    const double *src = A + (size_t)(c0 + i) + (size_t)(c0 + k) * lda;
    double v[36], q[8];
    {
        int b = 0;
#pragma unroll
        for (int ib = 0; ib < 8; ++ib)
#pragma unroll
            for (int kb = 0; kb <= ib; ++kb, ++b) {
                const double *sp = src + (size_t)(16 * ib) + (size_t)(16 * kb) * lda;
                v[b] = WT ? load_wt(sp) : *sp;
            }
    }
#pragma unroll
    for (int e = 0; e < 8; ++e) q[e] = WT ? load_wt(qin + tid + 256 * e) : qin[tid + 256 * e];
#pragma unroll
    for (int b = 0; b < 36; ++b) SL[b * 256 + k * 16 + i] = v[b];
#pragma unroll
    for (int e = 0; e < 8; ++e) QS[tid + 256 * e] = q[e];
}

__global__ void __launch_bounds__(256)
panel_pair_kernel(double *A, size_t lda, int c0, int r0, const double *q0, const double *q1, unsigned *out0, unsigned *xrw,
                  unsigned *out1, unsigned *abort_word, const double *mb0, const double *mb1,
                  double *smb, int nstrip, int npub, unsigned *sig, int sig_tile, double *xmb)
{
    __shared__ double SM[68 * 256];
    __shared__ int ok;
    double *SL = SM, *QS = SM + 36 * 256, *XS = SM;
    const int tid = threadIdx.x, lane = tid & 63, wave = tid >> 6;
    const int c1 = c0 + TILE;
    const bool split = xmb != nullptr;
    const int nfirst = split ? 2 * nstrip : nstrip;
    if ((int)blockIdx.x >= nfirst) {
        const int dd = (int)blockIdx.x - nfirst;
        const int ta = c_tri_ib[dd], tb = dd - ta * (ta + 1) / 2;
        const int rI = r0 + 64 * ta + 16 * wave, cJ = r0 + 64 * tb;
        d4 C[4], acc[4];
#pragma unroll
        for (int c = 0; c < 4; ++c) {
            C[c] = glb_blk(A, lda, rI, cJ + 16 * c, lane);
            acc[c] = (d4){0.0, 0.0, 0.0, 0.0};
        }
        const double *pi = smb + ((size_t)ta * 16 * 4 + wave) * 256 + lane;
        const double *pj = smb + ((size_t)tb * 16 * 4) * 256 + lane;
        double x[2][20];
#define DIAG_FETCH(kk, buf)                                                                                    \
        {                                                                                                      \
            _Pragma("unroll") for (int r = 0; r < 4; ++r) x[buf][r] = load_wt(pi + (size_t)(kk) * 1024 + 64 * r); \
            _Pragma("unroll") for (int c = 0; c < 4; ++c)                                                       \
                _Pragma("unroll") for (int r = 0; r < 4; ++r)                                                   \
                    x[buf][4 + 4 * c + r] = load_wt(pj + (size_t)(kk) * 1024 + 256 * c + 64 * r);                \
        }
        DIAG_FETCH(0, 0)
        bool good = true;
#pragma unroll
        for (int k = 0; k < 16; ++k) {
            const int cur = k & 1;
            for (unsigned it = 0; good; ++it) {
                bool missing = false;
#pragma unroll
                for (int e = 0; e < 20; ++e) missing = missing || __double_as_longlong(x[cur][e]) == -1ll;
                if (__builtin_amdgcn_ballot_w64(missing) == 0ull) break;
                const bool late_ = it > (unsigned)(ENGINE_TIMEOUT_TICKS / 100ull);
                if (late_ || ((it & 7u) == 7u && __hip_atomic_load(abort_word, __ATOMIC_RELAXED, __HIP_MEMORY_SCOPE_AGENT) != 0u)) {
                    if (late_ && lane == 0) __hip_atomic_store(abort_word, abort_code(ABORT_XCHG, (unsigned)(c0 / TILE)), __ATOMIC_RELAXED, __HIP_MEMORY_SCOPE_AGENT);
                    good = false;
                    break;
                }
                __builtin_amdgcn_s_sleep(2);
                if ((it & 7u) == 7u) {
#pragma unroll
                    for (int e = 0; e < 20; ++e)
                        if (__double_as_longlong(x[cur][e]) == -1ll) {
                            const double *ad = e < 4 ? pi + (size_t)k * 1024 + 64 * e
                                                     : pj + (size_t)k * 1024 + 256 * ((e - 4) >> 2) + 64 * ((e - 4) & 3);
                            x[cur][e] = __longlong_as_double((long long)__hip_atomic_fetch_or(
                                (unsigned long long *)const_cast<double *>(ad), 0ull, __ATOMIC_RELAXED, __HIP_MEMORY_SCOPE_AGENT));
                        }
                } else
                    DIAG_FETCH(k, cur)
            }
            if (k + 1 < 16) DIAG_FETCH(k + 1, cur ^ 1)
            d4 Xi = {x[cur][0], x[cur][1], x[cur][2], x[cur][3]};
#pragma unroll
            for (int c = 0; c < 4; ++c) {
                d4 Xj = {x[cur][4 + 4 * c], x[cur][5 + 4 * c], x[cur][6 + 4 * c], x[cur][7 + 4 * c]};
                blk_mma(acc[c], Xi, Xj);
            }
        }
#undef DIAG_FETCH
        if (tid == 0) ok = 1;
        __syncthreads();
        if (!good && lane == 0) ok = 0;
        __syncthreads();
        if (!ok) return;
#pragma unroll
        for (int c = 0; c < 4; ++c) glb_blk_store_wt(A, lda, rI, cJ + 16 * c, lane, C[c] - acc[c]);
        asm volatile("s_waitcnt vmcnt(0)" ::: "memory");
        __syncthreads();
        if (tid == 0) signal_add(sig + sig_tile + (ta >> 1));
        return;
    }
    const bool roleB = split && (int)blockIdx.x >= nstrip;
    const int strip = (int)blockIdx.x - (roleB ? nstrip : 0);
    const int rs = r0 + 64 * strip + 16 * wave;
    const bool pub = smb != nullptr && strip < npub;
    double *sp = smb + ((size_t)strip * 16 * 4 + wave) * 256;
    double *xp = split ? xmb + ((size_t)strip * 8 * 4 + wave) * 256 : nullptr;
    if (roleB) {
        int *okp = &ok;
        d4 B1[8], acc[8];
#pragma unroll
        for (int j = 0; j < 8; ++j) {
            B1[j] = glb_blk(A, lda, rs, c1 + 16 * j, lane);
            acc[j] = (d4){0.0, 0.0, 0.0, 0.0};
        }
        if (tid == 0) ok = wait_ge<false>(xrw, 1u, abort_word, abort_code(ABORT_INPANEL, (unsigned)(c0 / TILE))) ? 1 : 0;
        asm volatile("s_waitcnt vmcnt(0)" ::: "memory");
        __syncthreads();
        if (!ok) return;
        {
            const int i = tid & 15, k = tid >> 4;
            const double *Xg = A + (size_t)(c1 + i) + (size_t)(c0 + k) * lda;
            double st[2][16];
#pragma unroll
            for (int b = 0; b < 16; ++b) st[0][b] = load_wt(Xg + (size_t)(16 * (b >> 3)) + (size_t)(16 * (b & 7)) * lda);
#pragma unroll
            for (int r = 0; r < 4; ++r) {
                if (r + 1 < 4) {
#pragma unroll
                    for (int b = 0; b < 16; ++b) {
                        const int bb = 16 * (r + 1) + b;
                        st[(r + 1) & 1][b] = load_wt(Xg + (size_t)(16 * (bb >> 3)) + (size_t)(16 * (bb & 7)) * lda);
                    }
                }
#pragma unroll
                for (int b = 0; b < 16; ++b) XS[(16 * r + b) * 256 + k * 16 + i] = st[r & 1][b];
            }
        }
        __syncthreads();
        {
            const double *xq = xp + lane;
            double x[2][4];
#pragma unroll
            for (int r = 0; r < 4; ++r) x[0][r] = load_wt(xq + 64 * r);
            bool good = true;
#pragma unroll
            for (int kb = 0; kb < 8; ++kb) {
                const int cur = kb & 1;
                for (unsigned it = 0; good; ++it) {
                    bool missing = false;
#pragma unroll
                    for (int r = 0; r < 4; ++r) missing = missing || __double_as_longlong(x[cur][r]) == -1ll;
                    if (__builtin_amdgcn_ballot_w64(missing) == 0ull) break;
                    const bool late_ = it > (unsigned)(ENGINE_TIMEOUT_TICKS / 100ull);
                    if (late_ || ((it & 7u) == 7u && __hip_atomic_load(abort_word, __ATOMIC_RELAXED, __HIP_MEMORY_SCOPE_AGENT) != 0u)) {
                        if (late_ && lane == 0) __hip_atomic_store(abort_word, abort_code(ABORT_STRIPBOX, (unsigned)(c0 / TILE)), __ATOMIC_RELAXED, __HIP_MEMORY_SCOPE_AGENT);
                        good = false;
                        break;
                    }
                    __builtin_amdgcn_s_sleep(2);
#pragma unroll
                    for (int r = 0; r < 4; ++r) {
                        const double *ad = xq + (size_t)kb * 1024 + 64 * r;
                        if ((it & 7u) == 7u) {
                            if (__double_as_longlong(x[cur][r]) == -1ll)
                                x[cur][r] = __longlong_as_double((long long)__hip_atomic_fetch_or(
                                    (unsigned long long *)const_cast<double *>(ad), 0ull, __ATOMIC_RELAXED, __HIP_MEMORY_SCOPE_AGENT));
                        } else
                            x[cur][r] = load_wt(ad);
                    }
                }
                if (kb + 1 < 8) {
#pragma unroll
                    for (int r = 0; r < 4; ++r) x[cur ^ 1][r] = load_wt(xq + (size_t)(kb + 1) * 1024 + 64 * r);
                }
                if (good) {
#pragma unroll
                    for (int r = 0; r < 4; ++r) store_wt(const_cast<double *>(xq) + (size_t)kb * 1024 + 64 * r, __longlong_as_double(-1ll));
                }
                d4 Xk = {x[cur][0], x[cur][1], x[cur][2], x[cur][3]};
#pragma unroll
                for (int jj = 0; jj < 8; ++jj) {
                    d4 Xb = lds_blk(XS + (jj * 8 + kb) * 256, lane);
                    blk_mma(acc[jj], Xk, Xb);
                }
            }
            if (!good && lane == 0) ok = 0;
        }
#pragma unroll
        for (int jj = 0; jj < 8; ++jj) B1[jj] = B1[jj] - acc[jj];
        {
            const double *mb = mb1;
            double v9[3][9];
            __syncthreads();
            if (!ok) return;
            MBOX_FETCH256V(0, v9[0])
            MBOX_FETCH256V(1, v9[1])
#pragma unroll
            for (int j = 0; j < 8; ++j) {
                double *LS = SM + (j & 1) * (9 * 256);
                MBOX_COMPLETE256V(j, v9[j % 3], abort_word, abort_code(ABORT_PANEL, (unsigned)(c1 / TILE)))
#pragma unroll
                for (int i = 0; i < 9; ++i)
                    if (i <= 8 - j) LS[tid + 256 * i] = v9[j % 3][i];
                __syncthreads();
                if (!ok) return;
                if (j + 2 < 8) MBOX_FETCH256V(j + 2, v9[(j + 2) % 3])
                d4 L = lds_blk(LS, lane);
                double Q[4];
#pragma unroll
                for (int s = 0; s < 4; ++s) Q[s] = LS[(8 - j) * 256 + s * 64 + lane];
                trsm16(B1[j], L, Q);
                if (pub) mbox_store(sp + (size_t)(8 + j) * 1024, lane, B1[j]);
                d4 NX = -B1[j];
#pragma unroll
                for (int jj = j + 1; jj < 8; ++jj) {
                    d4 Lb = lds_blk(LS + (jj - j) * 256, lane);
                    blk_mma(B1[jj], NX, Lb);
                }
            }
        }
#pragma unroll
        for (int j = 0; j < 8; ++j) glb_blk_store(A, lda, rs, c1 + 16 * j, lane, B1[j]);
        return;
    }
    d4 B0[8], B1[8];
#pragma unroll
    for (int j = 0; j < 8; ++j) B0[j] = glb_blk(A, lda, rs, c0 + 16 * j, lane);
    if (!split) {
#pragma unroll
        for (int j = 0; j < 8; ++j) B1[j] = glb_blk(A, lda, rs, c1 + 16 * j, lane);
    }
    int *okp = &ok;
    if (mb0) {
        const double *mb = mb0;
        double v9[3][9];
        if (tid == 0) ok = 1;
        __syncthreads();
        MBOX_FETCH256V(0, v9[0])
        MBOX_FETCH256V(1, v9[1])
#pragma unroll
        for (int j = 0; j < 8; ++j) {
            double *LS = SM + (j & 1) * (9 * 256);
            MBOX_COMPLETE256V(j, v9[j % 3], abort_word, abort_code(ABORT_PANEL, (unsigned)(c0 / TILE)))
#pragma unroll
            for (int i = 0; i < 9; ++i)
                if (i <= 8 - j) LS[tid + 256 * i] = v9[j % 3][i];
            __syncthreads();
            if (!ok) return;
            if (j + 2 < 8) MBOX_FETCH256V(j + 2, v9[(j + 2) % 3])
            d4 L = lds_blk(LS, lane);
            double Q[4];
#pragma unroll
            for (int s = 0; s < 4; ++s) Q[s] = LS[(8 - j) * 256 + s * 64 + lane];
            trsm16(B0[j], L, Q);
            if (pub) mbox_store(sp + (size_t)j * 1024, lane, B0[j]);
            if (split) mbox_store(xp + (size_t)j * 1024, lane, B0[j]);
            d4 NX = -B0[j];
#pragma unroll
            for (int jj = j + 1; jj < 8; ++jj) {
                d4 Lb = lds_blk(LS + (jj - j) * 256, lane);
                blk_mma(B0[jj], NX, Lb);
            }
        }
    } else {
    if (tid == 0) ok = wait_ge<false>(out0, 1u, abort_word, abort_code(ABORT_PANEL, (unsigned)(c0 / TILE))) ? 1 : 0;
    asm volatile("s_waitcnt vmcnt(0)" ::: "memory");
    __syncthreads();
    if (!ok) return;
    fetch_factor_tile<true>(A, lda, c0, q0, SL, QS, tid);
    __syncthreads();
#pragma unroll
    for (int j = 0; j < 8; ++j) {
        d4 L = lds_blk(SL + (j * (j + 1) / 2 + j) * 256, lane);
        double Q[4];
#pragma unroll
        for (int s = 0; s < 4; ++s) Q[s] = QS[j * 256 + s * 64 + lane];
        trsm16(B0[j], L, Q);
        d4 NX = -B0[j];
#pragma unroll
        for (int jj = j + 1; jj < 8; ++jj) {
            d4 Lb = lds_blk(SL + (jj * (jj + 1) / 2 + j) * 256, lane);
            blk_mma(B0[jj], NX, Lb);
        }
    }
    }
#pragma unroll
    for (int j = 0; j < 8; ++j) glb_blk_store(A, lda, rs, c0 + 16 * j, lane, B0[j]);
    if (split) return;
    if (tid == 0) ok = wait_ge<false>(xrw, 1u, abort_word, abort_code(ABORT_INPANEL, (unsigned)(c0 / TILE))) ? 1 : 0;
    asm volatile("s_waitcnt vmcnt(0)" ::: "memory");
    __syncthreads();
    if (!ok) return;
    {
        const int i = tid & 15, k = tid >> 4;
        const double *Xg = A + (size_t)(c1 + i) + (size_t)(c0 + k) * lda;
        double st[2][16];
#pragma unroll
        for (int b = 0; b < 16; ++b) st[0][b] = load_wt(Xg + (size_t)(16 * (b >> 3)) + (size_t)(16 * (b & 7)) * lda);
#pragma unroll
        for (int r = 0; r < 4; ++r) {
            if (r + 1 < 4) {
#pragma unroll
                for (int b = 0; b < 16; ++b) {
                    const int bb = 16 * (r + 1) + b;
                    st[(r + 1) & 1][b] = load_wt(Xg + (size_t)(16 * (bb >> 3)) + (size_t)(16 * (bb & 7)) * lda);
                }
            }
#pragma unroll
            for (int b = 0; b < 16; ++b) XS[(16 * r + b) * 256 + k * 16 + i] = st[r & 1][b];
        }
        __syncthreads();
#pragma unroll
        for (int jj = 0; jj < 8; ++jj) {
            d4 acc = {0.0, 0.0, 0.0, 0.0};
#pragma unroll
            for (int kb = 0; kb < 8; ++kb) {
                d4 Xb = lds_blk(XS + (jj * 8 + kb) * 256, lane);
                blk_mma(acc, B0[kb], Xb);
            }
            B1[jj] = B1[jj] - acc;
        }
    }
    if (mb1) {
        const double *mb = mb1;
        double v9[3][9];
        __syncthreads();
        MBOX_FETCH256V(0, v9[0])
        MBOX_FETCH256V(1, v9[1])
#pragma unroll
        for (int j = 0; j < 8; ++j) {
            double *LS = SM + (j & 1) * (9 * 256);
            MBOX_COMPLETE256V(j, v9[j % 3], abort_word, abort_code(ABORT_PANEL, (unsigned)(c1 / TILE)))
#pragma unroll
            for (int i = 0; i < 9; ++i)
                if (i <= 8 - j) LS[tid + 256 * i] = v9[j % 3][i];
            __syncthreads();
            if (!ok) return;
            if (j + 2 < 8) MBOX_FETCH256V(j + 2, v9[(j + 2) % 3])
            d4 L = lds_blk(LS, lane);
            double Q[4];
#pragma unroll
            for (int s = 0; s < 4; ++s) Q[s] = LS[(8 - j) * 256 + s * 64 + lane];
            trsm16(B1[j], L, Q);
            if (pub) mbox_store(sp + (size_t)(8 + j) * 1024, lane, B1[j]);
            d4 NX = -B1[j];
#pragma unroll
            for (int jj = j + 1; jj < 8; ++jj) {
                d4 Lb = lds_blk(LS + (jj - j) * 256, lane);
                blk_mma(B1[jj], NX, Lb);
            }
        }
    } else {
    if (tid == 0) ok = wait_ge<false>(out1, 1u, abort_word, abort_code(ABORT_PANEL, (unsigned)(c1 / TILE))) ? 1 : 0;
    asm volatile("s_waitcnt vmcnt(0)" ::: "memory");
    __syncthreads();
    if (!ok) return;
    fetch_factor_tile<true>(A, lda, c1, q1, SL, QS, tid);
    __syncthreads();
#pragma unroll
    for (int j = 0; j < 8; ++j) {
        d4 L = lds_blk(SL + (j * (j + 1) / 2 + j) * 256, lane);
        double Q[4];
#pragma unroll
        for (int s = 0; s < 4; ++s) Q[s] = QS[j * 256 + s * 64 + lane];
        trsm16(B1[j], L, Q);
        d4 NX = -B1[j];
#pragma unroll
        for (int jj = j + 1; jj < 8; ++jj) {
            d4 Lb = lds_blk(SL + (jj * (jj + 1) / 2 + j) * 256, lane);
            blk_mma(B1[jj], NX, Lb);
        }
    }
    }
#pragma unroll
    for (int j = 0; j < 8; ++j) glb_blk_store(A, lda, rs, c1 + 16 * j, lane, B1[j]);
}

__global__ void __launch_bounds__(64)
engine_gate_kernel(unsigned *alive, unsigned *abort_word, unsigned code, unsigned long long ticks, unsigned nhelp,
                   unsigned *raise_in)
{
    if (threadIdx.x == 0) {
        bool ok = wait_ge<false>(alive, 1u, abort_word, code, ticks);
        if (ok && nhelp) ok = wait_ge<false>(alive + 2, nhelp, abort_word, code + 1u, ticks);
        if (ok && raise_in) {
            __hip_atomic_store(raise_in, 3u, __ATOMIC_RELAXED, __HIP_MEMORY_SCOPE_AGENT);
            __hip_atomic_store(raise_in + 1, 7u, __ATOMIC_RELAXED, __HIP_MEMORY_SCOPE_AGENT);
        }
    }
}

__global__ void __launch_bounds__(256)
trsm_tile_kernel(double *A, size_t lda, int c0, int r0, const double *qin, unsigned *wait_word, unsigned *abort_word,
                 int nb1, int e0, int own_world, int own_rank, int own_group)
{
    __shared__ double SL[36 * 256];
    __shared__ double QS[8 * 256];
    __shared__ int ok;
    const int tid = threadIdx.x, lane = tid & 63, wave = tid >> 6;
    if (own_world > 1) {
        const int row = (int)blockIdx.x < nb1 ? r0 + 64 * (int)blockIdx.x : e0 + 64 * ((int)blockIdx.x - nb1);
        if (((row / (2 * TILE) / own_group) % own_world) != own_rank) return;
    }
    if (wait_word) {
        if (tid == 0) ok = wait_ge<false>(wait_word, 1u, abort_word, abort_code(ABORT_PANEL, (unsigned)(c0 / TILE))) ? 1 : 0;
        asm volatile("s_waitcnt vmcnt(0)" ::: "memory");
        __syncthreads();
        if (!ok) return;
        fetch_factor_tile<true>(A, lda, c0, qin, SL, QS, tid);
    } else
        fetch_factor_tile<false>(A, lda, c0, qin, SL, QS, tid);
    const int bx = blockIdx.x;
    const int rs = (bx < nb1 ? r0 + 64 * bx : e0 + 64 * (bx - nb1)) + 16 * wave;
    d4 B[8];
#pragma unroll
    for (int j = 0; j < 8; ++j) B[j] = glb_blk(A, lda, rs, c0 + 16 * j, lane);
    __syncthreads();
#pragma unroll
    for (int j = 0; j < 8; ++j) {
        d4 L = lds_blk(SL + (j * (j + 1) / 2 + j) * 256, lane);
        double Q[4];
#pragma unroll
        for (int s = 0; s < 4; ++s) Q[s] = QS[j * 256 + s * 64 + lane];
        trsm16(B[j], L, Q);
        d4 NX = -B[j];
#pragma unroll
        for (int jj = j + 1; jj < 8; ++jj) {
            d4 Lb = lds_blk(SL + (jj * (jj + 1) / 2 + j) * 256, lane);
            blk_mma(B[jj], NX, Lb);
        }
    }
#pragma unroll
    for (int j = 0; j < 8; ++j) glb_blk_store(A, lda, rs, c0 + 16 * j, lane, B[j]);
}


struct UpdArgs {
    double *C; size_t ldc;
    const double *P; size_t ldp;
    int K;
    int ti0, tj0, lower_only;
    int H, W;
    unsigned *sig; int sig_tile;
    unsigned *wait_word, *abort_word;
    int ptiles, world, rank;
    const int *pmap;
    int skip_lo, skip_hi;
    unsigned *queue; unsigned ntiles;
    int Hb, ext0;
    int c_wt;
    int skew, kblk;
};

template <int TM, int KC, int ROLE, int NW = 4>
__global__ void __launch_bounds__(64 * NW, 8)
update_kernel(UpdArgs a)
{
    constexpr int LDT = TM + 16;
    constexpr int WY = NW / 2;
    constexpr int NB = TM / 32;
    constexpr int NBY = TM / WY / 16;
    constexpr int TPC = 64 * NW / KC;
    constexpr int RPT = TM / TPC;
    __shared__ double sI[2][KC * LDT];
    __shared__ double sJ[2][KC * LDT];
    unsigned *share = (unsigned *)&sI[0][TM];
    const int tid = threadIdx.x;
    const int wave_s = __builtin_amdgcn_readfirstlane(tid >> 6);
    if (a.wait_word) {
        if (tid == 0) *share = wait_ge(a.wait_word, 1u, a.abort_word, abort_code(ABORT_INPANEL, (unsigned)a.tj0)) ? 1u : 0u;
        asm volatile("s_waitcnt vmcnt(0)" ::: "memory");
        __syncthreads();
        const unsigned ok = *share;
        __syncthreads();
        if (!ok) return;
    }

    else if (a.abort_word) {
        if (tid == 0) *share = __hip_atomic_load(a.abort_word, __ATOMIC_RELAXED, __HIP_MEMORY_SCOPE_AGENT);
        __syncthreads();
        const unsigned ab = *share;
        __syncthreads();
        if (ab) return;
    }

    const int nch = a.K / KC;
    typedef double d2 __attribute__((ext_vector_type(2)));

    unsigned L = blockIdx.x;
    for (;;) {
        int lane;
        asm volatile("v_mbcnt_lo_u32_b32 %0, -1, 0\n\tv_mbcnt_hi_u32_b32 %0, -1, %0" : "=v"(lane));
        const int wave = wave_s, t2 = 64 * wave + lane;
        const int wi = wave & 1, wj = wave >> 1;
        const int kc = t2 / TPC, rg = (t2 % TPC) * RPT;
        const int ro = (lane >> 4) * LDT + (lane & 15);
        int ti, tj;
        if (a.lower_only) {
            int lo = 0, hi = a.W - 1;
            while (lo < hi) {
                const int mid = (lo + hi + 1) >> 1;
                if (mid * a.H - mid * (mid - 1) / 2 <= (int)L) lo = mid; else hi = mid - 1;
            }
            const int j = lo;
            const int til = j + ((int)L - (j * a.H - j * (j - 1) / 2));
            tj = a.tj0 + j;
            ti = til < a.Hb ? a.tj0 + til : a.ext0 + (til - a.Hb);
        } else {
            const int til = blockIdx.x;
            ti = til < a.Hb ? a.ti0 + til : a.ext0 + (til - a.Hb);
            tj = a.tj0 + blockIdx.y;
        }
        if (a.world > 1 && ((ti * TM / (2 * TILE) / a.ptiles) % a.world) != a.rank) return;
        if (ti >= a.skip_lo && ti < a.skip_hi && tj >= a.skip_lo && tj < a.skip_hi) {
            if (!a.queue) return;
            if (t2 == 0) *share = gridDim.x + __hip_atomic_fetch_add(a.queue, 1u, __ATOMIC_RELAXED, __HIP_MEMORY_SCOPE_AGENT);
            __syncthreads();
            L = (unsigned)__builtin_amdgcn_readfirstlane((int)*share);
            __syncthreads();
            if (L >= a.ntiles) break;
            continue;
        }
        const int sig_Ti = (ti * TM) / TILE - a.sig_tile, sig_Tj = (tj * TM) / TILE - a.sig_tile;
        const bool sig_wg = a.sig != nullptr && sig_Ti >= 0 && sig_Ti <= 1 && sig_Tj >= 0 && sig_Tj <= sig_Ti;
        const bool wt_wg = sig_wg || a.c_wt;
        if (sig_wg) __builtin_amdgcn_s_setprio(3); else __builtin_amdgcn_s_setprio(0);

        int rowI_P = ti * TM, rowJ_P = tj * TM, rowI_C = ti * TM;
        if (a.pmap) { rowI_P = a.pmap[ti]; rowJ_P = a.pmap[tj]; }
        if (a.skew) {
            const bool ext = ti >= a.ext0;
            const int under = a.skew * TILE + (ti - a.ext0) * TM;
            rowI_P = ext ? under : ti * TM - TILE * a.kblk;
            rowJ_P = tj * TM - TILE * a.kblk;
            rowI_C = ext ? under : ti * TM - TILE * ((tj * TM) / TILE);
        }
        const double *gI = a.P + (size_t)(rowI_P + rg) + (size_t)kc * a.ldp;
        const double *gJ = a.P + (size_t)(rowJ_P + rg) + (size_t)kc * a.ldp;
        d2 stI[RPT / 2], stJ[RPT / 2];

        double *Cb = a.C + (size_t)(rowI_C + (TM / 2) * wi) + (size_t)(tj * TM + (TM / WY) * wj) * a.ldc;
        const unsigned ldcb = 8u * (unsigned)a.ldc;
        const unsigned cvo = 8u * (unsigned)(lane & 15) + (unsigned)(lane >> 4) * ldcb;
        d4 acc[NB][NBY];
#pragma unroll
        for (int x = 0; x < NB; ++x)
#pragma unroll
            for (int y = 0; y < NBY; ++y) acc[x][y] = (d4){0.0, 0.0, 0.0, 0.0};

#pragma unroll
        for (int v = 0; v < RPT / 2; ++v) {
            stI[v] = *(const d2 *)(gI + 2 * v);
            stJ[v] = *(const d2 *)(gJ + 2 * v);
        }
#pragma unroll
        for (int v = 0; v < RPT / 2; ++v) {
            *(d2 *)(&sI[0][kc * LDT + rg + 2 * v]) = stI[v];
            *(d2 *)(&sJ[0][kc * LDT + rg + 2 * v]) = stJ[v];
        }
        __syncthreads();

        for (int ch = 0; ch < nch; ++ch) {
            const int cur = ch & 1;
            if (ch + 1 < nch) {
                const double *pI = gI + (size_t)(ch + 1) * KC * a.ldp;
                const double *pJ = gJ + (size_t)(ch + 1) * KC * a.ldp;
#pragma unroll
                for (int v = 0; v < RPT / 2; ++v) {
                    stI[v] = *(const d2 *)(pI + 2 * v);
                    stJ[v] = *(const d2 *)(pJ + 2 * v);
                }
            }
            const double *bI = &sI[cur][ro + (TM / 2) * wi];
            const double *bJ = &sJ[cur][ro + (TM / WY) * wj];
#pragma unroll
            for (int s = 0; s < KC / 4; ++s) {
                double pi_[NB], pj_[NBY];
#pragma unroll
                for (int x = 0; x < NB; ++x) pi_[x] = bI[s * 4 * LDT + 16 * x];
#pragma unroll
                for (int y = 0; y < NBY; ++y) pj_[y] = bJ[s * 4 * LDT + 16 * y];
#pragma unroll
                for (int x = 0; x < NB; ++x)
#pragma unroll
                    for (int y = 0; y < NBY; ++y) acc[x][y] = MFMA64(pj_[y], pi_[x], acc[x][y]);
            }
            if (ch + 1 < nch) {
#pragma unroll
                for (int v = 0; v < RPT / 2; ++v) {
                    *(d2 *)(&sI[cur ^ 1][kc * LDT + rg + 2 * v]) = stI[v];
                    *(d2 *)(&sJ[cur ^ 1][kc * LDT + rg + 2 * v]) = stJ[v];
                }
            }
            __syncthreads();
        }
        unsigned Lnext = 0;
        if (a.queue && t2 == 0)
            Lnext = gridDim.x + __hip_atomic_fetch_add(a.queue, 1u, __ATOMIC_RELAXED, __HIP_MEMORY_SCOPE_AGENT);
        unsigned cve = cvo;
        asm volatile("" : "+v"(cve));
#pragma unroll
        for (int x = 0; x < NB; ++x)
#pragma unroll
            for (int y = 0; y < NBY; ++y) {
                d4 cv;
#pragma unroll
                for (int r = 0; r < 4; ++r) {
                    const double *cp = (const double *)((const char *)(Cb + 16 * x) + (cve + (unsigned)(16 * y + 4 * r) * ldcb));
                    cv[r] = a.c_wt ? load_wt(cp) : *cp;
                }
                cv -= acc[x][y];
                if (wt_wg) {
#pragma unroll
                    for (int r = 0; r < 4; ++r)
                        store_wt((double *)((char *)(Cb + 16 * x) + (cve + (unsigned)(16 * y + 4 * r) * ldcb)), cv[r]);
                } else {
#pragma unroll
                    for (int r = 0; r < 4; ++r)
                        *(double *)((char *)(Cb + 16 * x) + (cve + (unsigned)(16 * y + 4 * r) * ldcb)) = cv[r];
                }
            }
        if (wt_wg) {
            asm volatile("s_waitcnt vmcnt(0)" ::: "memory");
            __syncthreads();
            if (t2 == 0 && sig_wg) signal_add(a.sig + a.sig_tile + sig_Ti);
        }
        if (!a.queue) break;
        if (t2 == 0) *share = Lnext;
        __syncthreads();
        L = (unsigned)__builtin_amdgcn_readfirstlane((int)*share);
        if (L >= a.ntiles) break;
    }
}

struct DagStep {
    unsigned base;
    unsigned near;
    unsigned tpos, nT;
    int H, W;
    int tj0;
    int k0, K;
    int nstrip, two;
    int need;
    int nd_next;
    int split;
    unsigned p2, p3;
};

struct DagArgs {
    double *A; size_t lda;
    double *P;
    const double *Wt;
    const DagStep *steps; int nsteps;
    unsigned ntasks;
    unsigned *queue;
    unsigned *tdone;
    unsigned *pdone; int pstride;
    unsigned *pall;
    double *partbuf;
    unsigned *dcount;
    unsigned *sig;
    unsigned *out, *xr;
    unsigned *abort_word;
    const unsigned *alive;
    unsigned xcc_quota;
    unsigned *hw;
    unsigned long long *trace;
    const unsigned *ftab;
    unsigned xcd_g;
    unsigned *xcnt;
};

constexpr unsigned DAG_XCD_LAG = 64u;
__device__ __forceinline__ unsigned dag_position(unsigned c, unsigned cls, unsigned g)
{
    return ((c >> g) << (g + 3u)) | (cls << g) | (c & ((1u << g) - 1u));
}

__device__ __forceinline__ bool dag_wait(const DagArgs &a, unsigned *word, unsigned need, unsigned code, unsigned L)
{
    const unsigned long long t0 = __builtin_amdgcn_s_memrealtime();
    for (unsigned it = 0;; ++it) {
        const unsigned v = poll_word(word, it);
        if (v >= need) break;
        if (__hip_atomic_load(a.abort_word, __ATOMIC_RELAXED, __HIP_MEMORY_SCOPE_AGENT) != 0u) return false;
        if (it > (unsigned)(ENGINE_TIMEOUT_TICKS / 100ull) ||
            ((it & 1023u) == 1023u && __builtin_amdgcn_s_memrealtime() - t0 > WALL_BACKSTOP_TICKS)) {
            if (__hip_atomic_exchange(a.abort_word, code, __ATOMIC_RELAXED, __HIP_MEMORY_SCOPE_AGENT) == 0u) {
                unsigned *d = a.queue + 8;
                d[0] = L; d[1] = code; d[2] = (unsigned)(word - a.queue); d[3] = need; d[4] = v;
                d[5] = (unsigned)(__builtin_amdgcn_s_memrealtime() - t0);
                d[6] = it;
            }
            return false;
        }
        __builtin_amdgcn_s_sleep(16);
    }
    __builtin_amdgcn_fence(__ATOMIC_ACQUIRE, "wavefront");
    return true;
}

__global__ void __launch_bounds__(256, 8)
dag_kernel(DagArgs a)
{
    constexpr int TM = 64, KC = 8, LDT = TM + 16, TPC = 256 / KC, RPT = TM / TPC;
    static_assert(RPT == 2, "one 16-byte load per thread, side and chunk");
    typedef double d2 __attribute__((ext_vector_type(2)));
    __shared__ double sI[2][KC * LDT];
    __shared__ double sJ[2][KC * LDT];
    unsigned *share = (unsigned *)&sI[0][TM];
    const int tid = threadIdx.x;
    const int wave_s = __builtin_amdgcn_readfirstlane(tid >> 6);
    const DagStep *__restrict__ steps = a.steps;
    const unsigned ldab = 8u * (unsigned)a.lda;
    int known = 0;
    const unsigned myx = (hw_where() >> 28) & 7u;
    const bool loyal = ((blockIdx.x >> 3) & 1u) == 0u;
    if (tid == 0) {
        bool take = true;
        if (a.xcc_quota) {
            const unsigned c = __hip_atomic_load(a.alive + 16 + myx, __ATOMIC_RELAXED, __HIP_MEMORY_SCOPE_AGENT);
            if (c) {
                const unsigned less = 7u * (c - 1u);
                const unsigned quota = a.xcc_quota > less + 8u ? a.xcc_quota - less : 8u;
                take = __hip_atomic_fetch_add(a.queue + 16 + myx, 1u, __ATOMIC_RELAXED, __HIP_MEMORY_SCOPE_AGENT) < quota;
            }
        }
        unsigned first = 0xffffffffu;
        if (take) {
            if (a.xcd_g) first = dag_position(__hip_atomic_fetch_add(a.xcnt + 32u * myx, 1u, __ATOMIC_RELAXED, __HIP_MEMORY_SCOPE_AGENT), myx, a.xcd_g);
            else first = __hip_atomic_fetch_add(a.queue, 1u, __ATOMIC_RELAXED, __HIP_MEMORY_SCOPE_AGENT);
        }
        share[1] = first;
        share[2] = 0u;
    }
    __syncthreads();
    unsigned L = (unsigned)__builtin_amdgcn_readfirstlane((int)share[1]);
    __syncthreads();
    if (L >= a.ntasks) return;
    for (;;) {
        int lo = 0, hi = a.nsteps - 1;
        while (lo < hi) {
            const int mid = (lo + hi + 1) >> 1;
            if (steps[mid].base <= L) lo = mid; else hi = mid - 1;
        }
        const int s = lo;
        const DagStep st = steps[s];
        const unsigned q = L - st.base;
        if (a.trace && tid == 0) {
            a.trace[4 * (size_t)L] = __builtin_amdgcn_s_memrealtime();
            if (a.hw) a.hw[2 * (size_t)L] = hw_where();
        }
        const int t = st.tj0 >> 1;
        const unsigned per_u = 2u * (unsigned)st.nstrip, nA = per_u + (unsigned)st.nd_next, perBC = st.two ? per_u : 0u;
        int tkind = -1;
        unsigned tu = 0, qt_u = q;
        if (q >= st.tpos) {
            if (q < st.tpos + nA) { tu = q - st.tpos; tkind = tu < per_u ? 0 : 3; }
            else if (q < st.p2) qt_u = q - nA;
            else if (q < st.p2 + perBC) { tu = q - st.p2; tkind = 1; }
            else if (q < st.p3) qt_u = q - nA - perBC;
            else if (q < st.p3 + perBC) { tu = q - st.p3; tkind = 2; }
            else qt_u = q - nA - 2u * perBC;
        }
        const bool isT = tkind >= 0;
        const double *gIb, *gJb;
        unsigned ldib, ldjb, ldob = ldab;
        int K, i_wt = 0, store_only = 0, strip_task = 0;
        double *Cb;
        const double *pa = nullptr;
        unsigned *w0 = nullptr, *w1 = nullptr, *w2 = nullptr, *we = nullptr, *we2 = nullptr, *dn;
        unsigned n0 = 0, n1 = 0, n2 = 0, ne = 0, dval = 0;
        int sigT = -1;
        int prio = 0;
        if (!isT) {
            const int qt = (int)qt_u;
            int ti, tj;
            if (a.ftab && qt >= (int)st.near) {
// ... 438 lines not shown
                blk_mma(acc[1][jb], P[1], Q);
            }
        }
    }
#pragma unroll
    for (int rb = 0; rb < 2; ++rb) {
        const int i = row0 + 16 * rb + (lane & 15);
        if (i >= n) continue;
        const double t = trend[i];
#pragma unroll
        for (int jb = 0; jb < 4; ++jb)
#pragma unroll
            for (int r = 0; r < 4; ++r) {
                const int j = s0 + 16 * jb + 4 * r + (lane >> 4);
                if (j < nsim) Y[(size_t)i + (size_t)j * ldy] = acc[rb][jb][r] + t;
            }
    }
}

static void set_dynamic_lds_once(const void *kernel, size_t bytes, std::atomic<unsigned long long> &done_mask);
void launch_band_trmm(const double *A, size_t lda, int skew, int npad, const int *d_hi, int nt, int n, const double *E,
                      int lde, int nsim, const double *trend, double *Y, int ldy, hipStream_t s)
{
    if (n <= 0 || nsim <= 0 || nt <= 0) return;
    static std::atomic<unsigned long long> attr_done{0};
    set_dynamic_lds_once((const void *)band_trmm_kernel, BT_LDS_BYTES, attr_done);
    hipLaunchKernelGGL(band_trmm_kernel, dim3(nt, (nsim + BT_COLS - 1) / BT_COLS), dim3(256), BT_LDS_BYTES, s,
                       A, lda, skew, npad, d_hi, n, E, lde, nsim, trend, Y, ldy);
}

__global__ void __launch_bounds__(256)
gather_rows_kernel(const double *Y, int ldy, const int *pos, int n, int ncol, double *out, int ldo)
{
    const int i = blockIdx.x * blockDim.x + threadIdx.x;
    if (i >= n) return;
    const int k = pos[i];
    for (int s = blockIdx.y; s < ncol; s += gridDim.y) out[(size_t)i + (size_t)s * ldo] = Y[(size_t)k + (size_t)s * ldy];
}

void launch_gather_rows(const double *Y, int ldy, const int *pos, int n, int ncol, double *out, int ldo, hipStream_t s)
{
    if (n <= 0 || ncol <= 0) return;
    const int gy = ncol < 64 ? ncol : 64;
    hipLaunchKernelGGL(gather_rows_kernel, dim3((n + 255) / 256, gy), dim3(256), 0, s, Y, ldy, pos, n, ncol, out, ldo);
}

static void set_dynamic_lds_once(const void *kernel, size_t bytes, std::atomic<unsigned long long> &done_mask)
{
    int dev = 0;
    (void)hipGetDevice(&dev);
    if (dev >= 0 && dev < 64 && ((done_mask.load(std::memory_order_relaxed) >> dev) & 1ull)) return;
    (void)hipFuncSetAttribute(kernel, hipFuncAttributeMaxDynamicSharedMemorySize, (int)bytes);
    if (dev >= 0 && dev < 64) done_mask.fetch_or(1ull << dev, std::memory_order_relaxed);
}

void launch_potrf_tile(double *A, size_t lda, int c0, double *dinv, int *info, hipStream_t s)
{
    const size_t shm = (36 + 1) * 256 * sizeof(double);
    static std::atomic<unsigned long long> attr_done{0};
    set_dynamic_lds_once((const void *)potrf_tile_kernel, shm, attr_done);
    hipLaunchKernelGGL(potrf_tile_kernel, dim3(1), dim3(512), shm, s, A, lda, c0, dinv, info);
}

__global__ void __launch_bounds__(64)
raise_word_kernel(unsigned *word)
{
    if (threadIdx.x == 0) __hip_atomic_store(word, 1u, __ATOMIC_RELAXED, __HIP_MEMORY_SCOPE_AGENT);
}

void launch_raise_word(unsigned *word, hipStream_t s) { hipLaunchKernelGGL(raise_word_kernel, dim3(1), dim3(64), 0, s, word); }

int streams_run_concurrently(hipStream_t first, hipStream_t second, unsigned *words)
{
    if (hipMemsetAsync(words, 0, 2 * sizeof(unsigned), second) != hipSuccess) return -1;
    if (hipStreamSynchronize(second) != hipSuccess) return -1;
    hipLaunchKernelGGL(engine_gate_kernel, dim3(1), dim3(64), 0, first, words, words + 1, 1u, 200000ull, 0u, (unsigned *)nullptr);
    hipLaunchKernelGGL(raise_word_kernel, dim3(1), dim3(64), 0, second, words);
    unsigned h[2] = {0, 0};
    if (hipStreamSynchronize(first) != hipSuccess || hipStreamSynchronize(second) != hipSuccess) return -1;
    if (hipMemcpyAsync(h, words, sizeof h, hipMemcpyDeviceToHost, second) != hipSuccess) return -1;
    if (hipStreamSynchronize(second) != hipSuccess) return -1;
    return h[1] == 0 ? 1 : 0;
}

void launch_engine_gate(unsigned *alive, unsigned *abort_word, hipStream_t s, bool last_tile, bool patient, int nhelp,
                        unsigned *raise_in)
{
    hipLaunchKernelGGL(engine_gate_kernel, dim3(1), dim3(64), 0, s, alive, abort_word, last_tile ? ABORT_LAST_TILE : ABORT_GATE,
                       last_tile ? ENGINE_TIMEOUT_TICKS : (patient ? 10 * GATE_TIMEOUT_TICKS : GATE_TIMEOUT_TICKS),
                       (unsigned)(last_tile || nhelp < 0 ? 0 : nhelp), last_tile ? nullptr : raise_in);
}

static size_t engine_lds_bytes()
{
    static size_t shm = 0;
    if (!shm) {
        shm = 150 * 1024;
        const char *x = getenv("COCONS_ENGINE_LDS");
        if (x && (size_t)atol(x) >= shm) shm = (size_t)atol(x);
    }
    return shm;
}

void launch_potrf_engine(double *A, size_t lda, int t0, int nt, double *dinv, int *info,
                         unsigned *in, unsigned *out, unsigned *xr, unsigned *abort_word, unsigned *alive, hipStream_t s,
                         double *wbuf, double *pbuf, int dag_until, unsigned long long *trace, double *mbox, int in_wait_ms)
{
    EngineArgs e;
    e.A = A; e.lda = lda; e.t0 = t0; e.nt = nt; e.dinv = dinv; e.info = info;
    e.in = in; e.out = out; e.xr = xr; e.abort_word = abort_word; e.alive = alive;
    e.wbuf = wbuf; e.pbuf = pbuf; e.dag_until = dag_until; e.trace = trace;
    e.in_ticks = in_wait_ms > 0 ? 100000ull * (unsigned long long)in_wait_ms : HOST_PACED_TICKS;
    e.mbox = mbox;
    e.partner = mbox ? 8 : 0;
    const int grid = e.partner ? e.partner + 1 : 1;
    const size_t shm = engine_lds_bytes();
    if (wbuf && pbuf) {
        static std::atomic<unsigned long long> attr_done{0};
        set_dynamic_lds_once((const void *)potrf_engine_kernel<true>, shm, attr_done);
        hipLaunchKernelGGL(potrf_engine_kernel<true>, dim3(grid), dim3(512), shm, s, e);
    } else {
        static std::atomic<unsigned long long> attr_done{0};
        set_dynamic_lds_once((const void *)potrf_engine_kernel<false>, shm, attr_done);
        hipLaunchKernelGGL(potrf_engine_kernel<false>, dim3(grid), dim3(512), shm, s, e);
    }
}

void launch_trsm_tile(double *A, size_t lda, int c0, int r0, int r1, const double *dinv, hipStream_t s,
                      unsigned *wait_word, unsigned *abort_word, int band_r1, int ext_r0, int own_world, int own_rank,
                      int own_group)
{
    int nb1 = ((band_r1 >= 0 ? band_r1 : r1) - r0) / 64, nb2 = band_r1 >= 0 ? (r1 - ext_r0) / 64 : 0;
    if (nb1 < 0) nb1 = 0;
    if (nb2 < 0) nb2 = 0;
    if (nb1 + nb2 <= 0) return;
    hipLaunchKernelGGL(trsm_tile_kernel, dim3(nb1 + nb2), dim3(256), 0, s, A, lda, c0, r0, dinv, wait_word, abort_word,
                       nb1, ext_r0, own_world, own_rank, own_group < 1 ? 1 : own_group);
}

void launch_potrf_follow(double *A, size_t lda, int c0, int r0, int r1, double *dinv, int *info, double *mbox,
                         unsigned *abort_word, hipStream_t s, int band_r1, int ext_r0)
{
    int nb1 = ((band_r1 >= 0 ? band_r1 : r1) - r0) / 64, nb2 = band_r1 >= 0 ? (r1 - ext_r0) / 64 : 0;
    if (nb1 < 0) nb1 = 0;
    if (nb2 < 0) nb2 = 0;
    const int nstrips = nb1 + nb2;
    static std::atomic<unsigned long long> attr_done{0};
    const size_t shm = 76 * 1024;
    set_dynamic_lds_once((const void *)potrf_follow_kernel, shm, attr_done);
    hipLaunchKernelGGL(potrf_follow_kernel, dim3(1 + (nstrips + 1) / 2), dim3(512), shm, s, A, lda, c0, dinv, info, mbox, r0, nb1,
                       ext_r0, nstrips, abort_word);
}

void launch_panel_pair(double *A, size_t lda, int c0, int r0, int r1, const double *q0, const double *q1, unsigned *out0,
                       unsigned *xr, unsigned *out1, unsigned *abort_word, hipStream_t s, const double *mb0, const double *mb1,
                       double *smb, int ndiag, unsigned *sig, int sig_tile, double *xmb)
{
    const int nb = (r1 - r0) / 64;
    if (nb <= 0) return;
    const bool split = xmb && mb0 && mb1;
    const bool diag = smb && mb0 && mb1 && ndiag > 0 && nb >= (ndiag == 10 ? 4 : 2);
    hipLaunchKernelGGL(panel_pair_kernel, dim3((split ? 2 * nb : nb) + (diag ? ndiag : 0)), dim3(256), 0, s, A, lda, c0, r0, q0, q1,
                       out0, xr, out1, abort_word, mb0, mb1, diag ? smb : nullptr, nb, diag ? (ndiag == 10 ? 4 : 2) : 0, sig, sig_tile,
                       split ? xmb : nullptr);
}

static int upd_waves = -1;
static long long upd_w8_max_tiles = -1;
void set_update_waves(int nw) { upd_waves = nw == 8 ? 8 : 4; }
void set_update_w8_max_tiles(int ntiles) { upd_w8_max_tiles = ntiles < 0 ? 0 : ntiles; }
static int upd_c_wt = 0;
void set_update_c_wt(int on) { upd_c_wt = on ? 1 : 0; }

void launch_update_from(double *A, size_t lda, const double *P, size_t ldp, int K,
                        int ti0, int ti1, int tj0, int tj1, bool lower_only, hipStream_t s,
                        int ptiles, int world, int rank, unsigned *sig, int sig_tile,
                        unsigned *wait_word, unsigned *abort_word, unsigned *queue, int band_hi, int ext0,
                        int skew, int kblk, int trim64, const int *pmap, int skip_lo, int skip_hi)
{
    const bool band = band_hi >= 0;
    const int rows_band = (band ? band_hi : ti1) - ti0, rows_ext = band ? ti1 - ext0 : 0;
    if (rows_band + rows_ext <= 0 || rows_band < 0 || rows_ext < 0 || tj1 <= tj0 || K <= 0) return;
    trim64 = trim64 ? 1 : 0;
    const int rows64 = 2 * (rows_band + rows_ext) - trim64;
    if (rows64 <= 0) return;
    if (upd_waves < 0) { const char *e = getenv("COCONS_UPD_WAVES"); set_update_waves(e ? atoi(e) : 8); }
    if (upd_w8_max_tiles < 0) { const char *e = getenv("COCONS_UPD_W8_MAX_TILES"); set_update_w8_max_tiles(e ? atoi(e) : 3500); }
    bool use_w8 = false;
    UpdArgs a;
    a.queue = nullptr; a.ntiles = 0;
    a.skew = skew; a.kblk = kblk; a.c_wt = upd_c_wt;
    a.Hb = 2 * rows_band; a.ext0 = 2 * ext0;
    a.C = A; a.ldc = lda; a.P = P; a.ldp = ldp; a.K = K;
    a.lower_only = lower_only ? 1 : 0;
    a.ptiles = ptiles < 1 ? 1 : ptiles; a.world = world; a.rank = rank; a.pmap = pmap; a.skip_lo = skip_lo; a.skip_hi = skip_hi;
    a.sig = sig; a.sig_tile = sig_tile;
    a.wait_word = wait_word; a.abort_word = abort_word;
    a.H = 0; a.W = 0;
    a.ti0 = 2 * ti0; a.tj0 = 2 * tj0;
    dim3 grid(rows64, 2 * (tj1 - tj0));
    if (lower_only) {
        if (ti0 != tj0) { a.lower_only = 0; }
        else {
            const long long H = rows64, W = 2LL * (tj1 - tj0);
            a.H = (int)H; a.W = (int)W;
            const long long total = W * H - W * (W - 1) / 2;
            static int slots = 0;
            if (!slots) {
                int dev = 0, cus = 256;
                hipGetDevice(&dev);
                hipDeviceGetAttribute(&cus, hipDeviceAttributeMultiprocessorCount, dev);
                slots = 8 * cus;
            }
            grid = dim3((unsigned)total, 1);
            if (queue && world == 1) {
                const bool w8 = upd_waves == 8 && K >= 2 * TILE && !skew &&
                                (upd_w8_max_tiles == 0 || total <= upd_w8_max_tiles);
                use_w8 = w8;
                const int cap = w8 ? slots / 2 - 4 : slots - 8;
                if (total > cap + (w8 ? 4 : 8)) {
                    a.queue = queue; a.ntiles = (unsigned)total;
                    grid = dim3((unsigned)cap, 1);
                }
            }
        }
    }
    const bool trailing = (K > TILE) && world == 1;
    if (trailing && use_w8 && a.lower_only) hipLaunchKernelGGL((update_kernel<64, 16, 0, 8>), grid, dim3(512), 0, s, a);
    else if (trailing) hipLaunchKernelGGL((update_kernel<64, 8, 0>), grid, dim3(256), 0, s, a);
    else hipLaunchKernelGGL((update_kernel<64, 8, 1>), grid, dim3(256), 0, s, a);
}

__global__ void __launch_bounds__(256)
pack_rows_kernel(const double *A, size_t lda, int col0, int ncols, double *dst, size_t ldp, const int *pmap, int ti_lo,
                 long long slot_lo, long long slot_hi)
{
    const int ti = ti_lo + (int)blockIdx.x;
    const long long off = pmap[ti];
    if (off < slot_lo || off >= slot_hi) return;
    const int rho = threadIdx.x & 63, cq = threadIdx.x >> 6;
    for (int c = 4 * (int)blockIdx.y + cq; c < ncols; c += 4 * (int)gridDim.y)
        dst[off + rho + (size_t)c * ldp] = A[(size_t)(64 * ti + rho) + (size_t)(col0 + c) * lda];
}

void launch_pack_rows(const double *A, size_t lda, int col0, int ncols, double *dst, size_t ldp, const int *pmap, int ti_lo,
                      int ti_hi, long long slot_lo, long long slot_hi, hipStream_t s)
{
    if (ti_hi <= ti_lo || ncols <= 0) return;
    hipLaunchKernelGGL(pack_rows_kernel, dim3(ti_hi - ti_lo, 8), dim3(256), 0, s, A, lda, col0, ncols, dst, ldp, pmap, ti_lo,
                       slot_lo, slot_hi);
}

static void dag_build_far_table(const std::vector<DagStepHost> &steps, std::vector<unsigned> &tab, int xcd_g, int bw, int bh)
{
    tab.assign(steps.size(), 0u);
    for (size_t s = 0; s < steps.size(); ++s) {
        const DagStepHost &st = steps[s];
        tab[s] = (unsigned)tab.size();
        const int nc = std::min(st.W, st.two ? 4 : 2);
        std::vector<std::vector<unsigned>> blocks;
        if (bw <= 0) {
            blocks.emplace_back();
            for (int jl = nc; jl < st.W; ++jl)
                for (int il = jl; il < st.H; ++il) blocks.back().push_back((unsigned)il << 16 | (unsigned)jl);
        } else {
            for (int c0 = nc; c0 < st.W; c0 += bw) {
                const int c1 = std::min(c0 + bw, st.W);
                for (int r0 = c0; r0 < st.H; r0 += bh) {
                    const int r1 = std::min(r0 + bh, st.H);
                    std::vector<unsigned> b;
                    for (int il = r0; il < r1; ++il)
                        for (int jl = c0; jl < c1 && jl <= il; ++jl) b.push_back((unsigned)il << 16 | (unsigned)jl);
                    if (!b.empty()) blocks.push_back(std::move(b));
                }
            }
        }
        const long long ntile = (long long)st.W * st.H - (long long)st.W * (st.W - 1) / 2;
        const long long nfar = ntile - st.near;
        const unsigned nA = 2u * (unsigned)st.nstrip + (unsigned)st.nd_next, perBC = st.two ? 2u * (unsigned)st.nstrip : 0u;
        const bool panels = st.nT > 0;
        size_t next_block = 0;
        size_t cur[8], pos_in[8];
        for (int x = 0; x < 8; ++x) { cur[x] = (size_t)-1; pos_in[x] = 0; }
        std::vector<size_t> taken_back(blocks.size(), 0);
        long long q = 0;
        const unsigned total = (unsigned)ntile + st.nT;
        for (unsigned pos = 0; pos < total && q < ntile; ++pos) {
            if (panels && ((pos >= st.tpos && pos < st.tpos + nA) || (pos >= st.p2 && pos < st.p2 + perBC) ||
                           (pos >= st.p3 && pos < st.p3 + perBC)))
                continue;
            const long long qt = q++;
            if (qt < (long long)st.near) continue;
            const int x = xcd_g > 0 ? (int)(((st.base + pos) >> xcd_g) & 7u) : 0;
            unsigned tile = 0;
            bool got = false;
            while (!got) {
                if (cur[x] != (size_t)-1 && pos_in[x] + taken_back[cur[x]] < blocks[cur[x]].size()) {
                    tile = blocks[cur[x]][pos_in[x]++];
                    got = true;
                } else if (next_block < blocks.size()) {
                    cur[x] = next_block++; pos_in[x] = 0;
                } else {
                    size_t best = (size_t)-1, left = 0;
                    for (int y = 0; y < 8; ++y)
                        if (cur[y] != (size_t)-1) {
                            const size_t l = blocks[cur[y]].size() - pos_in[y] - taken_back[cur[y]];
                            if (l > left) { left = l; best = cur[y]; }
                        }
                    if (best == (size_t)-1) break;
                    tile = blocks[best][blocks[best].size() - 1 - taken_back[best]++];
                    got = true;
                }
            }
            tab.push_back(tile);
        }
        (void)nfar;
    }
}

unsigned dag_build_steps(int nt, int mt, int trim64, int kskip, int lead, int min_tiles, int split, std::vector<DagStepHost> &out,
                         int lead2, int lead3, std::vector<unsigned> *ftab, int xcd_g, int bw, int bh)
{
    out.clear();
    if (ftab) ftab->clear();
    unsigned base = 0;
    int prev_two = 1;
    for (int k = 0; k + 2 < nt; k += 2) {
        const int t = k + 2;
        {
            const long long H0 = 2LL * (mt - t) - (trim64 ? 1 : 0), W0 = 2LL * (nt - t);
            if (W0 * H0 - W0 * (W0 - 1) / 2 < min_tiles) break;
        }
        DagStepHost st;
        st.tj0 = 2 * t;
        st.H = 2 * (mt - t) - (trim64 ? 1 : 0);
        st.W = 2 * (nt - t);
        st.two = t + 1 < nt ? 1 : 0;
        const long long tiles = (long long)st.W * st.H - (long long)st.W * (st.W - 1) / 2;
        const int nc = std::min(st.W, st.two ? 4 : 2);
        st.near = (unsigned)(nc * st.H - nc * (nc - 1) / 2);
        st.nstrip = std::max(0, st.H - (st.two ? 4 : 2));
        st.nT = (unsigned)(st.nstrip * (st.two ? 6 : 2));
        st.k0 = k * TILE + (k == 0 ? kskip : 0);
        st.K = 2 * TILE - (k == 0 ? kskip : 0);
        st.need = prev_two ? 6 : 2;
        st.nd_next = 0; st.split = 0;
        st.tpos = 0; st.p2 = 0; st.p3 = 0;
        st.base = 0;
        prev_two = st.two;
        (void)tiles;
        out.push_back(st);
    }
    if (!out.empty()) {
        DagStepHost &l = out.back();
        l.nT = 0; l.nstrip = 0;
    }
    if (split)
        for (size_t s = 0; s + 1 < out.size(); ++s)
            if (out[s].nstrip > 0 && out[s].two) {
                out[s].nd_next = out[s + 1].two ? 10 : 3;
                out[s + 1].split = 1;
            }
    for (auto &st : out) {
        const long long ntile = (long long)st.W * st.H - (long long)st.W * (st.W - 1) / 2;
        st.nT += (unsigned)st.nd_next;
        const long long nA = 2LL * st.nstrip + st.nd_next;
        const long long perBC = st.two ? 2LL * st.nstrip : 0;
        const long long far = ntile - st.near;
        st.tpos = st.near + (unsigned)std::min<long long>(far, lead);
        st.base = base;
        base += (unsigned)ntile + st.nT;
        long long rem = ntile - (long long)st.tpos;
        if (st.nT == 0) { st.p2 = st.p3 = st.tpos; continue; }
        const long long d2 = std::min<long long>(rem, perBC ? lead2 : 0);
        rem -= d2;
        const long long d3 = std::min<long long>(rem, perBC ? lead3 : 0);
        st.p2 = (unsigned)(st.tpos + nA + d2);
        st.p3 = (unsigned)(st.p2 + perBC + d3);
    }
    if (ftab) dag_build_far_table(out, *ftab, xcd_g, bw, bh);
    return base;
}

void launch_dag(double *A, size_t lda, double *P, const double *Wt, const DagStepHost *dsteps, int nsteps, unsigned ntasks,
                unsigned *queue, unsigned *tdone, unsigned *pdone, int pstride, unsigned *pall, double *partbuf, unsigned *dcount,
                unsigned *sig, unsigned *out, unsigned *xr, unsigned *abort_word, hipStream_t s, unsigned long long *trace,
                const unsigned *alive, int xcc_quota, unsigned *hw, const unsigned *ftab, int xcd_g, unsigned *xcnt)
{
    static_assert(sizeof(DagStepHost) == sizeof(DagStep), "host and device step records");
    if (nsteps <= 0 || ntasks == 0) return;
    DagArgs a;
    a.A = A; a.lda = lda; a.P = P; a.Wt = Wt;
    a.steps = (const DagStep *)dsteps; a.nsteps = nsteps; a.ntasks = ntasks;
    a.queue = queue; a.tdone = tdone; a.pdone = pdone; a.pstride = pstride; a.pall = pall;
    a.partbuf = partbuf; a.dcount = dcount;
    a.sig = sig; a.out = out; a.xr = xr; a.abort_word = abort_word; a.trace = trace; a.hw = trace ? hw : nullptr;
    static int slots = 0;
    if (!slots) {
        int dev = 0, cus = 256;
        hipGetDevice(&dev);
        hipDeviceGetAttribute(&cus, hipDeviceAttributeMultiprocessorCount, dev);
        slots = 8 * cus;
    }
    const unsigned cap = (unsigned)(slots - 8);
    a.alive = alive; a.xcc_quota = (alive && xcc_quota > 0) ? (unsigned)xcc_quota : 0u;
    a.ftab = ftab; a.xcd_g = (ftab && xcnt && xcd_g > 0) ? (unsigned)xcd_g : 0u;
    a.xcnt = xcnt;
    hipLaunchKernelGGL(dag_kernel, dim3(ntasks < cap ? ntasks : cap), dim3(256), 0, s, a);
}

void launch_update(double *A, size_t lda, int k0, int K, int ti0, int ti1, int tj0, int tj1,
                   bool lower_only, hipStream_t s, unsigned *sig, int sig_tile,
                   unsigned *wait_word, unsigned *abort_word, unsigned *queue, int band_hi, int ext0,
                   int skew, int trim64, int skip_lo, int skip_hi)
{
    launch_update_from(A, lda, A + (size_t)k0 * lda, lda, K, ti0, ti1, tj0, tj1, lower_only, s, 1, 1, 0, sig, sig_tile,
                       wait_word, abort_word, queue, band_hi, ext0, skew, k0 / TILE, trim64, nullptr, skip_lo, skip_hi);
}

void launch_finalize_cols(const double *A, size_t lda, int c0, int c1, int n, int row0, int nr,
                          double *out, hipStream_t s)
{
    hipLaunchKernelGGL(finalize_kernel, dim3(nr * nr + 1), dim3(1024), 0, s, A, lda, c0, c1, n, row0, nr, out, 0, 0,
                       (const double *)nullptr, 0);
}

void launch_finalize(const double *A, size_t lda, int n, int row0, int nr, double *out, hipStream_t s, int skew, int npad,
                     const double *A2, int a2_cols)
{
    hipLaunchKernelGGL(finalize_kernel, dim3(nr * nr + 1), dim3(1024), 0, s, A, lda, 0, n, n, row0, nr, out, skew, npad,
                       skew ? (const double *)nullptr : A2, a2_cols);
}

size_t row_reduce_scratch_doubles(int n, int m)
{
    return (size_t)2 * (size_t)m * (size_t)((n + 255) / 256);
}

void launch_row_reduce(const double *A, size_t lda, int n, int rowy, int row0, int m,
                       double *stoch, double *quad, double *scratch, hipStream_t s, int skew, int npad,
                       const double *A2, int a2_cols)
{
    if (m <= 0) return;
    const int cchunk = 2 * TILE, nchunks = (n + cchunk - 1) / cchunk;
    hipLaunchKernelGGL(row_reduce_kernel, dim3((m + 255) / 256, nchunks), dim3(256), 0, s,
                       A, lda, n, rowy, row0, m, scratch, cchunk, skew, npad, skew ? (const double *)nullptr : A2, a2_cols);
    hipLaunchKernelGGL(row_reduce_final_kernel, dim3((m + 255) / 256), dim3(256), 0, s,
                       scratch, m, nchunks, stoch, quad);
}



__device__ __forceinline__ void krige_tile_ij(int t, int &I, int &J)
{
    int i = (int)((sqrt(8.0 * t + 1.0) - 1.0) * 0.5);
    while ((i + 1) * (i + 2) / 2 <= t) ++i;
    while (i * (i + 1) / 2 > t) --i;
    I = i; J = t - i * (i + 1) / 2;
}

__global__ void __launch_bounds__(256)
krige_pack_kernel(const double *A, size_t lda, double *Lp)
{
    int I, J;
    krige_tile_ij((int)blockIdx.x, I, J);
    const double *src = A + (size_t)I * TILE + (size_t)J * TILE * lda;
    double *dst = Lp + (size_t)blockIdx.x * TILE * TILE;
    for (int e = threadIdx.x; e < TILE * TILE; e += 256) {
        const int r = e & (TILE - 1), c = e >> 7;
        const double v = src[(size_t)r + (size_t)c * lda];
        dst[e] = (I == J && r < c) ? 0.0 : v;
    }
}

__global__ void __launch_bounds__(256)
krige_qprep_kernel(const double *A, size_t lda, int rowy, int c_lo, int c_hi, double *Qp, double *w)
{
    const int J = blockIdx.x, tid = threadIdx.x;
    if (tid < TILE) {
        const int c = J * TILE + tid;
        w[c] = (c >= c_lo && c < c_hi) ? A[(size_t)rowy + (size_t)c * lda] : 0.0;
    }
    for (int e = tid; e < 8 * 256; e += 256) {
        const int jb = e >> 8, s = (e >> 6) & 3, lane = e & 63;
        const int m = lane & 15, k = lane >> 4, c = m & 3;
        double q = 0.0;
        if ((m >> 2) == s && k <= c) {
            const double *L = A + (size_t)(J * TILE + 16 * jb + 4 * s) * (1 + lda);
            const double l10 = L[1], l20 = L[2], l30 = L[3], l21 = L[2 + lda], l31 = L[3 + lda], l32 = L[3 + 2 * lda];
            const double r0 = 1.0 / L[0], r1 = 1.0 / L[1 + lda], r2 = 1.0 / L[2 + 2 * lda], r3 = 1.0 / L[3 + 3 * lda];
            const double m00 = r0, m11 = r1, m22 = r2, m33 = r3;
            const double m10 = -(l10 * m00) * r1;
            const double m21 = -(l21 * m11) * r2;
            const double m32 = -(l32 * m22) * r3;
            const double m20 = -fma(l21, m10, l20 * m00) * r2;
            const double m31 = -fma(l32, m21, l31 * m11) * r3;
            const double m30 = -fma(l32, m20, fma(l31, m10, l30 * m00)) * r3;
            q = sel_lower4(c, k, m00, m10, m11, m20, m21, m22, m30, m31, m32, m33);
        }
        Qp[(size_t)J * 2048 + e] = q;
    }
}

__global__ void __launch_bounds__(256)
krige_diag_kernel(const double *Lp, const double *Qp, const double *w, double *C, size_t ldc, int J, int c_lo, int c_hi,
                  double *stoch, double *quad)
{
    __shared__ double SL[36 * 256];
    __shared__ double QS[8 * 256];
    const int tid = threadIdx.x, lane = tid & 63, wave = tid >> 6;
    fetch_factor_tile<false>(Lp + (size_t)(J * (J + 1) / 2 + J) * TILE * TILE, TILE, 0, Qp + (size_t)J * 2048, SL, QS, tid);
    const int rs = 64 * (int)blockIdx.x + 16 * wave, c0 = J * TILE;
    d4 B[8];
#pragma unroll
    for (int j = 0; j < 8; ++j) {
        B[j] = glb_blk(C, ldc, rs, c0 + 16 * j, lane);
#pragma unroll
        for (int r = 0; r < 4; ++r) {
            const int c = c0 + 16 * j + 4 * r + (lane >> 4);
            if (c < c_lo || c >= c_hi) B[j][r] = 0.0;
        }
    }
    __syncthreads();
#pragma unroll
    for (int j = 0; j < 8; ++j) {
        d4 L = lds_blk(SL + (j * (j + 1) / 2 + j) * 256, lane);
        double Q[4];
#pragma unroll
        for (int s = 0; s < 4; ++s) Q[s] = QS[j * 256 + s * 64 + lane];
        trsm16(B[j], L, Q);
        d4 NX = -B[j];
#pragma unroll
        for (int jj = j + 1; jj < 8; ++jj) {
            d4 Lb = lds_blk(SL + (jj * (jj + 1) / 2 + j) * 256, lane);
            blk_mma(B[jj], NX, Lb);
        }
    }
    double sp = 0.0, qp = 0.0;
#pragma unroll
    for (int j = 0; j < 8; ++j)
#pragma unroll
        for (int r = 0; r < 4; ++r) {
            const int c = c0 + 16 * j + 4 * r + (lane >> 4);
            const double v = (c < c_lo || c >= c_hi) ? 0.0 : B[j][r];
            B[j][r] = v;
            sp = fma(v, w[c], sp);
            qp = fma(v, v, qp);
        }
    sp += __shfl_xor(sp, 16);
    qp += __shfl_xor(qp, 16);
    sp += __shfl_xor(sp, 32);
    qp += __shfl_xor(qp, 32);
    if (lane < 16) {
        const int i = rs + lane;
        if (J == 0) { stoch[i] = sp; quad[i] = qp; }
        else { stoch[i] += sp; quad[i] += qp; }
    }
#pragma unroll
    for (int j = 0; j < 8; ++j) glb_blk_store(C, ldc, rs, c0 + 16 * j, lane, B[j]);
}

constexpr int KU_KC = 32;
__global__ void __launch_bounds__(256)
krige_update_kernel(const double *Lp, double *C, size_t ldc, int J)
{
    __shared__ double LS[TILE * KU_KC];
    const int tid = threadIdx.x, lane = tid & 63, wave = tid >> 6;
    const int I = J + 1 + (int)blockIdx.y;
    const double *Lt = Lp + (size_t)(I * (I + 1) / 2 + J) * TILE * TILE;
    const int rs = 64 * (int)blockIdx.x + 16 * wave;
// ... 54 lines not shown
```

cocons_amd/csrc/kernels.h:

```cpp
#pragma once
#include <hip/hip_runtime.h>
#include <stddef.h>
#include <vector>
#include "../../include/cocons_hip.h"

namespace cocons {

enum SmoothKind : int {
    SMOOTH_ZERO = 0,
    SMOOTH_LOGISTIC_SQRT = 1,
    SMOOTH_EXP = 2
};

struct ThetaVecs {
    double tilt[COCONS_P_MAX];
    double two_scale_je[COCONS_P_MAX];
    double aniso[COCONS_P_MAX];
    double sqrt_vector[COCONS_P_MAX];
    double half_sd[COCONS_P_MAX];
    double nugget[COCONS_P_MAX];
    double smooth[COCONS_P_MAX];
    double sd[COCONS_P_MAX];
};

struct LocArgs {
    int n, p;
    const double *X; int ldx;
    const double *locs; int ldl;
    double *out; size_t stride;
    int smooth_kind;
    double smooth_min, smooth_max;
    ThetaVecs th;
};

struct PairArgs {
    int n;
    int m;
    const double *rows;
    const double *cols;
    size_t stride;
    size_t stride_rows;
    double *out; size_t ld;
    int nrows_out, ncols_out;
    int bj0;
    int H;
    int blocked;
    double gr;
    double nu_fixed;
    double pad_diag;
    int own_world = 0, own_rank = 0, own_group = 1;
};

struct RhsArgs {
    int n, p;
    const double *X; int ldx;
    double mean[COCONS_P_MAX];
    int use_trend;
    const double *src; int lds;
    double *out; size_t ld;
    int row0, nrows;
    int nrows_zero;
    int col0, ncols_out;
    int skew, npad;
};

void launch_loc_params(const LocArgs &a, hipStream_t s);
void launch_pair_sym(int mode, bool mirror, const PairArgs &a, hipStream_t s);
void launch_pair_rect(int mode, const PairArgs &a, hipStream_t s);
void launch_rhs_rows(const RhsArgs &a, hipStream_t s);
void launch_taper(int mode, bool pred, int nrows, int nnz, const int *ci, const int *rp, const double *rows,
                  size_t stride_rows, const double *cols, size_t stride, double nu_fixed, double *out, hipStream_t s,
                  const double *tapv = nullptr, double *A = nullptr, size_t lda = 0, int row0 = 0,
                  int skew = 0, int npad = 0);
void launch_band_zero(double *A, size_t lda, const int *d_hi, int nt, int max_band, hipStream_t s, int skew = 0);
void launch_front_identity(double *A, size_t lda, int pad0, int rows, hipStream_t s);
void launch_pad_identity(double *A, size_t lda, int n, int npad, hipStream_t s, int skew = 0);
void launch_cov_rows(int mode, int n, int nidx, const int *idx, const double *loc, size_t stride, double gr,
                     double nu_fixed, int cor, double *out, hipStream_t s);
void launch_matern_points(int n, const double *nu, const double *x, double *out, hipStream_t s);

constexpr int TILE = 128;

__host__ __device__ inline size_t band_index(int i, int j, size_t ld, int skew, int npad)
{
    if (skew == 0) return (size_t)i + (size_t)j * ld;
    const int il = i < npad ? i - TILE * (j / TILE) : skew * TILE + (i - npad);
    return (size_t)il + (size_t)j * ld;
}
inline double *band_base(double *A, int c, int skew) { return skew ? A - (ptrdiff_t)TILE * c : A; }

void launch_potrf_tile(double *A, size_t lda, int c0, double *dinv, int *info, hipStream_t s);
void launch_potrf_follow(double *A, size_t lda, int c0, int r0, int r1, double *dinv, int *info, double *mbox,
                         unsigned *abort_word, hipStream_t s, int band_r1 = -1, int ext_r0 = 0);
void launch_potrf_engine(double *A, size_t lda, int t0, int nt, double *dinv, int *info,
                         unsigned *in, unsigned *out, unsigned *xr, unsigned *abort_word, unsigned *alive, hipStream_t s,
                         double *wbuf = nullptr, double *pbuf = nullptr, int dag_until = 0,
                         unsigned long long *trace = nullptr,
                         double *mbox = nullptr,
                         int in_wait_ms = 0);
constexpr unsigned ABORT_ENGINE_IN0 = 0x100u, ABORT_ENGINE_IN1 = 0x200u, ABORT_PANEL = 0x300u, ABORT_XCHG = 0x400u, ABORT_INPANEL = 0x500u,
                   ABORT_GATE = 0x600u, ABORT_PARTNER = 0x700u, ABORT_FOLLOW = 0x800u, ABORT_LAST_TILE = 0x900u, ABORT_STRIPBOX = 0xf00u,
                   ABORT_DAG_FIRST = 0xa00u, ABORT_DAG_LAST = 0xe00u;
__host__ __device__ inline unsigned abort_code(unsigned cls, unsigned index) { return cls | (index & 0xffu); }
inline unsigned abort_class(unsigned code) { return code & 0xf00u; }
constexpr size_t ENGINE_MBOX_DOUBLES = 44 * 256;
void launch_engine_gate(unsigned *alive, unsigned *abort_word, hipStream_t s, bool last_tile = false, bool patient = false, int nhelp = 0,
                        unsigned *raise_in = nullptr);
void launch_raise_word(unsigned *word, hipStream_t s);
int streams_run_concurrently(hipStream_t first, hipStream_t second, unsigned *words);
void launch_trsm_tile(double *A, size_t lda, int c0, int r0, int r1, const double *dinv, hipStream_t s,
                      unsigned *wait_word = nullptr, unsigned *abort_word = nullptr, int band_r1 = -1, int ext_r0 = 0,
                      int own_world = 0, int own_rank = 0, int own_group = 1);
void launch_panel_pair(double *A, size_t lda, int c0, int r0, int r1, const double *q0, const double *q1, unsigned *out0,
                       unsigned *xr, unsigned *out1, unsigned *abort_word, hipStream_t s, const double *mb0 = nullptr,
                       const double *mb1 = nullptr,
                       double *smb = nullptr, int ndiag = 0, unsigned *sig = nullptr, int sig_tile = 0,
                       double *xmb = nullptr);
constexpr size_t PANEL_XMBOX_DOUBLES = 8 * 4 * 256;
constexpr size_t PANEL_SMBOX_DOUBLES = 4 * 16 * 4 * 256;
void launch_update(double *A, size_t lda, int k0, int K, int ti0, int ti1, int tj0, int tj1,
                   bool lower_only, hipStream_t s, unsigned *sig = nullptr, int sig_tile = -1,
                   unsigned *wait_word = nullptr, unsigned *abort_word = nullptr, unsigned *queue = nullptr,
                   int band_hi = -1, int ext0 = 0,
                   int skew = 0,
                   int trim64 = 0,
                   int skip_lo = 0, int skip_hi = 0);
void set_update_waves(int nw);
void set_update_w8_max_tiles(int ntiles);
void set_update_c_wt(int on);
void launch_update_from(double *A, size_t lda, const double *P, size_t ldp, int K,
                        int ti0, int ti1, int tj0, int tj1, bool lower_only, hipStream_t s,
                        int group, int world, int rank, unsigned *sig = nullptr, int sig_tile = -1,
                        unsigned *wait_word = nullptr, unsigned *abort_word = nullptr, unsigned *queue = nullptr,
                        int band_hi = -1, int ext0 = 0, int skew = 0, int kblk = 0, int trim64 = 0,
                        const int *pmap = nullptr, int skip_lo = 0, int skip_hi = 0);
void launch_pack_rows(const double *A, size_t lda, int col0, int ncols, double *dst, size_t ldp, const int *pmap, int ti_lo,
                      int ti_hi, long long slot_lo, long long slot_hi, hipStream_t s);

struct DagStepHost {
    unsigned base, near, tpos, nT;
    int H, W, tj0, k0, K, nstrip, two, need, nd_next, split;
    unsigned p2, p3;
};
unsigned dag_build_steps(int nt, int mt, int trim64, int kskip, int lead, int min_tiles, int split, std::vector<DagStepHost> &out,
                         int lead2 = 0, int lead3 = 0,
                         std::vector<unsigned> *ftab = nullptr,
                         int xcd_g = 0, int bw = 16, int bh = 16);
void launch_dag(double *A, size_t lda, double *P, const double *Wt, const DagStepHost *dsteps, int nsteps, unsigned ntasks,
                unsigned *queue, unsigned *tdone, unsigned *pdone, int pstride, unsigned *pall, double *partbuf, unsigned *dcount,
                unsigned *sig, unsigned *out, unsigned *xr, unsigned *abort_word, hipStream_t s, unsigned long long *trace = nullptr,
                const unsigned *alive = nullptr, int xcc_quota = 0, unsigned *hw = nullptr,
                const unsigned *ftab = nullptr, int xcd_g = 0,
                unsigned *xcnt = nullptr);

void launch_finalize(const double *A, size_t lda, int n, int row0, int nr, double *out, hipStream_t s,
                     int skew = 0, int npad = 0,
                     const double *A2 = nullptr,
                     int a2_cols = 0);
void launch_finalize_cols(const double *A, size_t lda, int c0, int c1, int n, int row0, int nr,
                          double *out, hipStream_t s);
size_t row_reduce_scratch_doubles(int n, int m);
void launch_row_reduce(const double *A, size_t lda, int n, int rowy, int row0, int m,
                       double *stoch, double *quad, double *scratch, hipStream_t s, int skew = 0, int npad = 0,
                       const double *A2 = nullptr, int a2_cols = 0);

void launch_trmm_lower(const double *A, size_t lda, int n, const double *E, int lde, int nsim,
                       const double *trend, double *Y, int ldy, hipStream_t s);
void launch_band_trmm(const double *A, size_t lda, int skew, int npad, const int *d_hi, int nt, int n, const double *E,
                      int lde, int nsim, const double *trend, double *Y, int ldy, hipStream_t s);
void launch_krige_pack(const double *A, size_t lda, int nt, int rowy, int c_lo, int c_hi, double *Lp, double *Qp, double *w,
                       hipStream_t s);
void launch_krige_solve(const double *Lp, const double *Qp, const double *w, int nt, double *C, size_t ldc, int rows,
                        int c_lo, int c_hi, double *stoch, double *quad, hipStream_t s);
void launch_gather_rows(const double *Y, int ldy, const int *pos, int n, int ncol, double *out, int ldo, hipStream_t s);

}
```

Before: 120.8.

## Add tail lookahead: launch panel on third stream once near-panel update tiles finish

In the tail loop after the DAG phase, the trailing update kernel now counts completions of the 64-row tiles that feed the next panel into a per-step 'near' flag. A new third stream waits on that counter with hipStreamWaitValue32 and launches the panel_pair kernel early, using write-through loads and stores, while the rest of the trailing update is still running. The main stream then waits on a done counter before continuing. This is meant to take the panel off the critical path of each tail step. It adds stream-creation probing, larger flag buffers, and a risk of deadlock if the streams do not actually run concurrently.

```diff
diff --git a/cocons_amd/csrc/api.hip b/cocons_amd/csrc/api.hip
--- a/cocons_amd/csrc/api.hip
+++ b/cocons_amd/csrc/api.hip
@@ -315,6 +315,7 @@
     bool xbuf_own;
     hipEvent_t ev[8];
     hipStream_t stream2;
+    hipStream_t stream3;
     hipEvent_t ev_eng;
     unsigned *dflags;
     int flags_cap;
@@ -471,6 +472,7 @@
         if (f->taper_twin) { cocons_fit_destroy(f->taper_twin); f->taper_twin = nullptr; }
         delete f->krige; f->krige = nullptr;
         if (f->stream2) hipStreamDestroy(f->stream2);
+        if (f->stream3) hipStreamDestroy(f->stream3);
         if (f->own_stream && f->stream) hipStreamDestroy(f->stream);
     }
     delete f->h_locs; delete f->h_X; delete f->h_z; delete f->h_xb;
@@ -1035,6 +1037,7 @@
     int panel_split = 32;
     int panel_diag = 1;
     int potrf_follow = 1;
+    int tail_lookahead = 1;
     int dag_trace = 0;
     int gate_sabotage = 0;
     int host_delay_us = 0, host_delay_tile = -1, engine_in_wait_ms = 0;
@@ -1065,6 +1068,7 @@
         rd("COCONS_PANEL_FOLLOW", t.panel_follow);
         rd("COCONS_PANEL_DIAG", t.panel_diag);
         rd("COCONS_PANEL_SPLIT", t.panel_split);
+        rd("COCONS_TAIL_LOOKAHEAD", t.tail_lookahead);
         rd("COCONS_DEBUG_HOST_DELAY_US", t.host_delay_us);
         rd("COCONS_DEBUG_HOST_DELAY_TILE", t.host_delay_tile);
         t.init = true;
@@ -1105,6 +1109,7 @@
     else if (k == "panel_follow") t.panel_follow = value;
     else if (k == "panel_diag") t.panel_diag = value;
     else if (k == "panel_split") t.panel_split = value;
+    else if (k == "tail_lookahead") t.tail_lookahead = value;
     else if (k == "gate_sabotage") t.gate_sabotage = value;
     else if (k == "host_delay_us") t.host_delay_us = value;
     else if (k == "host_delay_tile") t.host_delay_tile = value;
@@ -1144,7 +1149,8 @@
 
 static void timed_update(cocons_fit *f, const FactorView &v, int k, int kw, int t0, int t1, hipStream_t s,
                          std::vector<hipEvent_t> *ev_upd, unsigned *sig, int sig_tile, unsigned *queue = nullptr,
-                         int skip_tiles = 0)
+                         int skip_tiles = 0,
+                         unsigned *near = nullptr)
 {
     const int mt = v.mt;
     if (t1 <= t0) return;
@@ -1159,7 +1165,8 @@
     }
     const int kskip = (k == 0 && !v.hi) ? (f->pad0 / 16) * 16 : 0;
     launch_update(v.A, v.lda, k * TILE + kskip, kw * TILE - kskip, t0, mt, t0, t1, true, s, sig, sig_tile, nullptr,
-                  abort_word, queue, hb, v.nt, 0, v.trim, skip_tiles > 0 ? 2 * t0 : 0, skip_tiles > 0 ? 2 * (t0 + skip_tiles) : 0);
+                  abort_word, queue, hb, v.nt, 0, v.trim, skip_tiles > 0 ? 2 * t0 : 0, skip_tiles > 0 ? 2 * (t0 + skip_tiles) : 0,
+                  near, t0);
     if (ev_upd) {
         hipEventRecord(b, s);
         ev_upd->push_back(a); ev_upd->push_back(b);
@@ -1180,15 +1187,22 @@
     return engine_enabled() && f->engine_ok && f->stream2 != nullptr && f->engine_skip == 0 && v.nt > 4;
 }
 
+static size_t flags_words(int cap) { return 4 * (size_t)cap + 64 + ((size_t)cap + 4) * 32; }
+static unsigned *la_near(cocons_fit *f, int k) { return f->dflags + 4 * (size_t)f->flags_cap + 64 + (size_t)(k / 2) * 32; }
+static unsigned *la_done(cocons_fit *f, int t)
+{
+    return f->dflags + 4 * (size_t)f->flags_cap + 64 + ((size_t)f->flags_cap / 2 + 2 + (size_t)(t / 2)) * 32;
+}
+
 static int flags_reset(cocons_fit *f, int nt)
 {
     if (f->flags_cap < nt) {
         if (f->stream2) HIPCHK(hipStreamSynchronize(f->stream2));
         if (f->dflags) { HIPCHK(hipFree(f->dflags)); f->dflags = nullptr; }
         f->flags_cap = round_up(nt + 8, 64);
-        HIPCHK(hipMalloc(&f->dflags, (4 * (size_t)f->flags_cap + 64) * sizeof(unsigned)));
-    }
-    HIPCHK(hipMemsetAsync(f->dflags, 0, (4 * (size_t)f->flags_cap + 64) * sizeof(unsigned), f->stream));
+        HIPCHK(hipMalloc(&f->dflags, flags_words(f->flags_cap) * sizeof(unsigned)));
+    }
+    HIPCHK(hipMemsetAsync(f->dflags, 0, flags_words(f->flags_cap) * sizeof(unsigned), f->stream));
     return 0;
 }
 
@@ -1287,7 +1301,22 @@
         for (hipStream_t l : losers) hipStreamDestroy(l);
         if (ok < 0) { (void)hipGetLastError(); return fail(-100, "engine_warm: stream self-test failed"); }
         if (ok == 0) { f->engine_ok = false; return 0; }
-        HIPCHK(hipMemsetAsync(f->dflags, 0, (4 * (size_t)f->flags_cap + 64) * sizeof(unsigned), f->stream));
+        int wait_value = 0;
+        (void)hipDeviceGetAttribute(&wait_value, hipDeviceAttributeCanUseStreamWaitValue, f->device);
+        if (!f->stream3 && wait_value) {
+            std::vector<hipStream_t> spare;
+            for (int attempt = 0; attempt < 4; ++attempt) {
+                if (hipStreamCreateWithFlags(&f->stream3, hipStreamNonBlocking) != hipSuccess) { f->stream3 = nullptr; break; }
+                const int a = streams_run_concurrently(f->stream2, f->stream3, words);
+                const int b = a == 1 ? streams_run_concurrently(f->stream3, f->stream, words) : a;
+                if (a < 0 || b < 0) { (void)hipGetLastError(); hipStreamDestroy(f->stream3); f->stream3 = nullptr; break; }
+                if (a == 1 && b == 1) break;
+                spare.push_back(f->stream3);
+                f->stream3 = nullptr;
+            }
+            for (hipStream_t l : spare) hipStreamDestroy(l);
+        }
+        HIPCHK(hipMemsetAsync(f->dflags, 0, flags_words(f->flags_cap) * sizeof(unsigned), f->stream));
         HIPCHK(hipStreamSynchronize(f->stream));
     }
     launch_potrf_engine(nullptr, 0, 0, 0, f->dinv, f->dinfo, f->dflags, f->dflags, f->dflags, (unsigned *)(f->dinfo + 1),
@@ -1429,6 +1458,7 @@
         if (int rc = mbox_reset(f, nt > f->nt ? nt : f->nt)) return rc;
     HIPCHK(hipEventRecord(f->ev_eng, M));
     HIPCHK(hipStreamWaitEvent(f->stream2, f->ev_eng, 0));
+    if (f->stream3) HIPCHK(hipStreamWaitEvent(f->stream3, f->ev_eng, 0));
     unsigned *alive_w = f->dflags + 3 * (size_t)f->flags_cap;
     f->engine_t0 = (tun().engine_block0 && !v.hi) ? 0 : 2;
     launch_potrf_engine(v.A, v.lda, f->engine_t0, nt, f->dinv, f->dinfo, in, out, xr, (unsigned *)(f->dinfo + 1),
@@ -1486,7 +1516,7 @@
                        f->engine_pair_live,
                        (block0 && tun().gate_sabotage == 0 && alive == f->dflags + 3 * (size_t)f->flags_cap) ? in : nullptr);
     const int rend = mt * TILE - 64 * v.trim;
-    auto panel_for = [&](int t, bool allow_diag) -> int {
+    auto panel_for = [&](int t, bool allow_diag, hipStream_t ps = nullptr, unsigned *done = nullptr, int *nwg = nullptr) -> int {
         const bool two = t + 1 < nt;
         const int r0 = two ? t + 2 : t + 1;
         const int hb = band_hi(v, t);
@@ -1499,12 +1529,14 @@
             const int nstrips = (rend - r0 * TILE) / 64;
             const bool sp = fol && tun().panel_split > 0 && nstrips >= tun().panel_split &&
                             (size_t)nstrips * PANEL_XMBOX_DOUBLES <= f->xmb_elems;
-            launch_panel_pair(v.A, v.lda, t * TILE, r0 * TILE, rend, f->dinv + (size_t)(t & 1) * 2048,
-                              f->dinv + (size_t)((t + 1) & 1) * 2048, out + t, xr + t, out + t + 1, abort_word, M,
-                              fol ? f->dmbox + (size_t)t * ENGINE_MBOX_DOUBLES : nullptr,
-                              fol ? f->dmbox + (size_t)(t + 1) * ENGINE_MBOX_DOUBLES : nullptr,
-                              dg ? f->dmbox + f->smb_off + (size_t)(t >> 1) * PANEL_SMBOX_DOUBLES : nullptr,
-                              dg ? (next_tiles == 2 ? 10 : 3) : 0, in, t + 2, sp ? f->dmbox + f->xmb_off : nullptr);
+            const int launched =
+                launch_panel_pair(v.A, v.lda, t * TILE, r0 * TILE, rend, f->dinv + (size_t)(t & 1) * 2048,
+                                  f->dinv + (size_t)((t + 1) & 1) * 2048, out + t, xr + t, out + t + 1, abort_word, ps ? ps : M,
+                                  fol ? f->dmbox + (size_t)t * ENGINE_MBOX_DOUBLES : nullptr,
+                                  fol ? f->dmbox + (size_t)(t + 1) * ENGINE_MBOX_DOUBLES : nullptr,
+                                  dg ? f->dmbox + f->smb_off + (size_t)(t >> 1) * PANEL_SMBOX_DOUBLES : nullptr,
+                                  dg ? (next_tiles == 2 ? 10 : 3) : 0, in, t + 2, sp ? f->dmbox + f->xmb_off : nullptr, done);
+            if (nwg) *nwg = launched;
             return (dg && nstrips >= (next_tiles == 2 ? 4 : 2)) ? next_tiles : 0;
         }
         launch_trsm_tile(v.A, v.lda, t * TILE, r0 * TILE, rend, f->dinv + (size_t)(t & 1) * 2048, M,
@@ -1542,14 +1574,32 @@
         if (ev_upd) { hipEventRecord(eb, M); ev_upd->push_back(ea); ev_upd->push_back(eb); f->dag_events = 1; }
         k_first = 2 * f->dag_nsteps;
     }
+    const bool la_on = tun().tail_lookahead != 0 && f->stream3 != nullptr && !v.hi && tun().panel_fused;
     for (int k = k_first > 0 ? k_first - 2 : 0; k + 2 < nt; k += 2) {
         const int t = k + 2;
         if (tun().host_delay_us > 0 && t + 2 == tun().host_delay_tile) usleep((useconds_t)tun().host_delay_us);
+        unsigned *near = nullptr;
+        unsigned need = 0;
+        if (la_on && k >= k_first && t + 1 < nt && band_hi(v, t) < 0) {
+            const int rows64 = 2 * (mt - t) - v.trim, cols64 = 2 * (nt - t);
+            if (rows64 > 4) {
+                need = 4u * (unsigned)(rows64 - 4);
+                const int rc = rows64 < 8 ? rows64 : 8, wc = cols64 < 8 ? cols64 : 8;
+                for (int j = 4; j < wc; ++j) need += (unsigned)(rc > j ? rc - j : 0);
+                near = la_near(f, k);
+            }
+        }
         if (k >= k_first) {
             if (ev_upd) count_update_flops(f, 2, t);
-            timed_update(f, v, k, 2, t, nt, M, ev_upd, in, t, tile_queue(f, k), diag_done);
-        }
-        diag_done = panel_for(t, k + 4 < nt);
+            timed_update(f, v, k, 2, t, nt, M, ev_upd, in, t, tile_queue(f, k), diag_done, near);
+        }
+        if (near) {
+            HIPCHK(hipStreamWaitValue32(f->stream3, near, need, hipStreamWaitValueGte, 0xffffffffu));
+            int nwg = 0;
+            diag_done = panel_for(t, k + 4 < nt, f->stream3, la_done(f, t), &nwg);
+            if (nwg > 0) HIPCHK(hipStreamWaitValue32(M, la_done(f, t), (unsigned)nwg, hipStreamWaitValueGte, 0xffffffffu));
+        } else
+            diag_done = panel_for(t, k + 4 < nt);
     }
     if (mt == nt) launch_engine_gate(out + (nt - 1), abort_word, M, true);
     return 0;
@@ -1808,7 +1858,7 @@
     }
     for (hipStream_t l : losers) hipStreamDestroy(l);
     if (c->stream2 && streams_run_concurrently(c->stream2, c->stream, words) == 0) c->engine_ok = false;
-    (void)hipMemsetAsync(c->dflags, 0, (4 * (size_t)c->flags_cap + 64) * sizeof(unsigned), c->stream);
+    (void)hipMemsetAsync(c->dflags, 0, flags_words(c->flags_cap) * sizeof(unsigned), c->stream);
     (void)hipStreamSynchronize(c->stream);
 }
 
diff --git a/cocons_amd/csrc/chol.hip b/cocons_amd/csrc/chol.hip
--- a/cocons_amd/csrc/chol.hip
+++ b/cocons_amd/csrc/chol.hip
@@ -891,8 +891,21 @@
     for (int e = 0; e < 8; ++e) QS[tid + 256 * e] = q[e];
 }
 
-__global__ void __launch_bounds__(256)
-panel_pair_kernel(double *A, size_t lda, int c0, int r0, const double *q0, const double *q1, unsigned *out0, unsigned *xrw,
+template <bool LA>
+__device__ __forceinline__ d4 pp_load(const double *A, size_t lda, int row0, int col0, int lane)
+{
+    return LA ? glb_blk_wt(A, lda, row0, col0, lane) : glb_blk(A, lda, row0, col0, lane);
+}
+template <bool LA>
+__device__ __forceinline__ void pp_store(double *A, size_t lda, int row0, int col0, int lane, const d4 &v)
+{
+    if (LA) glb_blk_store_wt(A, lda, row0, col0, lane, v);
+    else glb_blk_store(A, lda, row0, col0, lane, v);
+}
+
+template <bool LA>
+__device__ __forceinline__ void
+panel_pair_body(double *A, size_t lda, int c0, int r0, const double *q0, const double *q1, unsigned *out0, unsigned *xrw,
                   unsigned *out1, unsigned *abort_word, const double *mb0, const double *mb1,
                   double *smb, int nstrip, int npub, unsigned *sig, int sig_tile, double *xmb)
 {
@@ -910,7 +923,7 @@
         d4 C[4], acc[4];
 #pragma unroll
         for (int c = 0; c < 4; ++c) {
-            C[c] = glb_blk(A, lda, rI, cJ + 16 * c, lane);
+            C[c] = pp_load<LA>(A, lda, rI, cJ + 16 * c, lane);
             acc[c] = (d4){0.0, 0.0, 0.0, 0.0};
         }
         const double *pi = smb + ((size_t)ta * 16 * 4 + wave) * 256 + lane;
@@ -984,7 +997,7 @@
         d4 B1[8], acc[8];
 #pragma unroll
         for (int j = 0; j < 8; ++j) {
-            B1[j] = glb_blk(A, lda, rs, c1 + 16 * j, lane);
+            B1[j] = pp_load<LA>(A, lda, rs, c1 + 16 * j, lane);
             acc[j] = (d4){0.0, 0.0, 0.0, 0.0};
         }
         if (tid == 0) ok = wait_ge<false>(xrw, 1u, abort_word, abort_code(ABORT_INPANEL, (unsigned)(c0 / TILE))) ? 1 : 0;
@@ -1094,15 +1107,15 @@
             }
         }
 #pragma unroll
-        for (int j = 0; j < 8; ++j) glb_blk_store(A, lda, rs, c1 + 16 * j, lane, B1[j]);
+        for (int j = 0; j < 8; ++j) pp_store<LA>(A, lda, rs, c1 + 16 * j, lane, B1[j]);
         return;
     }
     d4 B0[8], B1[8];
 #pragma unroll
-    for (int j = 0; j < 8; ++j) B0[j] = glb_blk(A, lda, rs, c0 + 16 * j, lane);
+    for (int j = 0; j < 8; ++j) B0[j] = pp_load<LA>(A, lda, rs, c0 + 16 * j, lane);
     if (!split) {
 #pragma unroll
-        for (int j = 0; j < 8; ++j) B1[j] = glb_blk(A, lda, rs, c1 + 16 * j, lane);
+        for (int j = 0; j < 8; ++j) B1[j] = pp_load<LA>(A, lda, rs, c1 + 16 * j, lane);
     }
     int *okp = &ok;
     if (mb0) {
@@ -1159,7 +1172,7 @@
     }
     }
 #pragma unroll
-    for (int j = 0; j < 8; ++j) glb_blk_store(A, lda, rs, c0 + 16 * j, lane, B0[j]);
+    for (int j = 0; j < 8; ++j) pp_store<LA>(A, lda, rs, c0 + 16 * j, lane, B0[j]);
     if (split) return;
     if (tid == 0) ok = wait_ge<false>(xrw, 1u, abort_word, abort_code(ABORT_INPANEL, (unsigned)(c0 / TILE))) ? 1 : 0;
     asm volatile("s_waitcnt vmcnt(0)" ::: "memory");
@@ -1247,7 +1260,21 @@
     }
     }
 #pragma unroll
-    for (int j = 0; j < 8; ++j) glb_blk_store(A, lda, rs, c1 + 16 * j, lane, B1[j]);
+    for (int j = 0; j < 8; ++j) pp_store<LA>(A, lda, rs, c1 + 16 * j, lane, B1[j]);
+}
+
+template <bool LA>
+__global__ void __launch_bounds__(256)
+panel_pair_kernel(double *A, size_t lda, int c0, int r0, const double *q0, const double *q1, unsigned *out0, unsigned *xrw,
+                  unsigned *out1, unsigned *abort_word, const double *mb0, const double *mb1,
+                  double *smb, int nstrip, int npub, unsigned *sig, int sig_tile, double *xmb, unsigned *done)
+{
+    panel_pair_body<LA>(A, lda, c0, r0, q0, q1, out0, xrw, out1, abort_word, mb0, mb1, smb, nstrip, npub, sig, sig_tile, xmb);
+    if (LA) {
+        asm volatile("s_waitcnt vmcnt(0)" ::: "memory");
+        __syncthreads();
+        if (threadIdx.x == 0) signal_add(done);
+    }
 }
 
 __global__ void __launch_bounds__(64)
@@ -1324,7 +1351,9 @@
     int Hb, ext0;
     int c_wt;
     int skew, kblk;
+    unsigned *near; int near_lo;
 };
+constexpr unsigned NEAR_RELEASE = 1u << 16;
 
 template <int TM, int KC, int ROLE, int NW = 4>
 __global__ void __launch_bounds__(64 * NW, 8)
@@ -1355,7 +1384,10 @@
         __syncthreads();
         const unsigned ab = *share;
         __syncthreads();
-        if (ab) return;
+        if (ab) {
+            if (a.near && tid == 0) __hip_atomic_fetch_add(a.near, NEAR_RELEASE, __ATOMIC_RELAXED, __HIP_MEMORY_SCOPE_AGENT);
+            return;
+        }
     }
 
     const int nch = a.K / KC;
@@ -1397,7 +1429,9 @@
         }
         const int sig_Ti = (ti * TM) / TILE - a.sig_tile, sig_Tj = (tj * TM) / TILE - a.sig_tile;
         const bool sig_wg = a.sig != nullptr && sig_Ti >= 0 && sig_Ti <= 1 && sig_Tj >= 0 && sig_Tj <= sig_Ti;
-        const bool wt_wg = sig_wg || a.c_wt;
+        const int nr_j = tj - a.near_lo;
+        const bool near_wg = a.near != nullptr && nr_j >= 0 && ((nr_j < 4 && ti >= a.near_lo + 4) || (nr_j < 8 && ti < a.near_lo + 8 && nr_j >= 4));
+        const bool wt_wg = sig_wg || near_wg || a.c_wt;
         if (sig_wg) __builtin_amdgcn_s_setprio(3); else __builtin_amdgcn_s_setprio(0);
 
         int rowI_P = ti * TM, rowJ_P = tj * TM, rowI_C = ti * TM;
@@ -1498,6 +1532,7 @@
             asm volatile("s_waitcnt vmcnt(0)" ::: "memory");
             __syncthreads();
             if (t2 == 0 && sig_wg) signal_add(a.sig + a.sig_tile + sig_Ti);
+            if (t2 == 0 && near_wg) signal_add(a.near);
         }
         if (!a.queue) break;
         if (t2 == 0) *share = Lnext;
@@ -2242,17 +2277,24 @@
                        ext_r0, nstrips, abort_word);
 }
 
-void launch_panel_pair(double *A, size_t lda, int c0, int r0, int r1, const double *q0, const double *q1, unsigned *out0,
-                       unsigned *xr, unsigned *out1, unsigned *abort_word, hipStream_t s, const double *mb0, const double *mb1,
-                       double *smb, int ndiag, unsigned *sig, int sig_tile, double *xmb)
+int launch_panel_pair(double *A, size_t lda, int c0, int r0, int r1, const double *q0, const double *q1, unsigned *out0,
+                      unsigned *xr, unsigned *out1, unsigned *abort_word, hipStream_t s, const double *mb0, const double *mb1,
+                      double *smb, int ndiag, unsigned *sig, int sig_tile, double *xmb, unsigned *done)
 {
     const int nb = (r1 - r0) / 64;
-    if (nb <= 0) return;
+    if (nb <= 0) return 0;
     const bool split = xmb && mb0 && mb1;
     const bool diag = smb && mb0 && mb1 && ndiag > 0 && nb >= (ndiag == 10 ? 4 : 2);
-    hipLaunchKernelGGL(panel_pair_kernel, dim3((split ? 2 * nb : nb) + (diag ? ndiag : 0)), dim3(256), 0, s, A, lda, c0, r0, q0, q1,
-                       out0, xr, out1, abort_word, mb0, mb1, diag ? smb : nullptr, nb, diag ? (ndiag == 10 ? 4 : 2) : 0, sig, sig_tile,
-                       split ? xmb : nullptr);
+    const int nwg = (split ? 2 * nb : nb) + (diag ? ndiag : 0);
+    if (done)
+        hipLaunchKernelGGL(panel_pair_kernel<true>, dim3(nwg), dim3(256), 0, s, A, lda, c0, r0, q0, q1, out0, xr, out1, abort_word,
+                           mb0, mb1, diag ? smb : nullptr, nb, diag ? (ndiag == 10 ? 4 : 2) : 0, sig, sig_tile, split ? xmb : nullptr,
+                           done);
+    else
+        hipLaunchKernelGGL(panel_pair_kernel<false>, dim3(nwg), dim3(256), 0, s, A, lda, c0, r0, q0, q1, out0, xr, out1, abort_word,
+                           mb0, mb1, diag ? smb : nullptr, nb, diag ? (ndiag == 10 ? 4 : 2) : 0, sig, sig_tile, split ? xmb : nullptr,
+                           nullptr);
+    return nwg;
 }
 
 static int upd_waves = -1;
@@ -2266,7 +2308,7 @@
                         int ti0, int ti1, int tj0, int tj1, bool lower_only, hipStream_t s,
                         int ptiles, int world, int rank, unsigned *sig, int sig_tile,
                         unsigned *wait_word, unsigned *abort_word, unsigned *queue, int band_hi, int ext0,
-                        int skew, int kblk, int trim64, const int *pmap, int skip_lo, int skip_hi)
+                        int skew, int kblk, int trim64, const int *pmap, int skip_lo, int skip_hi, unsigned *near, int near_lo)
 {
     const bool band = band_hi >= 0;
     const int rows_band = (band ? band_hi : ti1) - ti0, rows_ext = band ? ti1 - ext0 : 0;
@@ -2286,6 +2328,7 @@
     a.ptiles = ptiles < 1 ? 1 : ptiles; a.world = world; a.rank = rank; a.pmap = pmap; a.skip_lo = skip_lo; a.skip_hi = skip_hi;
     a.sig = sig; a.sig_tile = sig_tile;
     a.wait_word = wait_word; a.abort_word = abort_word;
+    a.near = near; a.near_lo = 2 * near_lo;
     a.H = 0; a.W = 0;
     a.ti0 = 2 * ti0; a.tj0 = 2 * tj0;
     dim3 grid(rows64, 2 * (tj1 - tj0));
@@ -2502,10 +2545,10 @@
 void launch_update(double *A, size_t lda, int k0, int K, int ti0, int ti1, int tj0, int tj1,
                    bool lower_only, hipStream_t s, unsigned *sig, int sig_tile,
                    unsigned *wait_word, unsigned *abort_word, unsigned *queue, int band_hi, int ext0,
-                   int skew, int trim64, int skip_lo, int skip_hi)
+                   int skew, int trim64, int skip_lo, int skip_hi, unsigned *near, int near_lo)
 {
     launch_update_from(A, lda, A + (size_t)k0 * lda, lda, K, ti0, ti1, tj0, tj1, lower_only, s, 1, 1, 0, sig, sig_tile,
-                       wait_word, abort_word, queue, band_hi, ext0, skew, k0 / TILE, trim64, nullptr, skip_lo, skip_hi);
+                       wait_word, abort_word, queue, band_hi, ext0, skew, k0 / TILE, trim64, nullptr, skip_lo, skip_hi, near, near_lo);
 }
 
 void launch_finalize_cols(const double *A, size_t lda, int c0, int c1, int n, int row0, int nr,
diff --git a/cocons_amd/csrc/kernels.h b/cocons_amd/csrc/kernels.h
--- a/cocons_amd/csrc/kernels.h
+++ b/cocons_amd/csrc/kernels.h
@@ -111,11 +111,12 @@
 void launch_trsm_tile(double *A, size_t lda, int c0, int r0, int r1, const double *dinv, hipStream_t s,
                       unsigned *wait_word = nullptr, unsigned *abort_word = nullptr, int band_r1 = -1, int ext_r0 = 0,
                       int own_world = 0, int own_rank = 0, int own_group = 1);
-void launch_panel_pair(double *A, size_t lda, int c0, int r0, int r1, const double *q0, const double *q1, unsigned *out0,
-                       unsigned *xr, unsigned *out1, unsigned *abort_word, hipStream_t s, const double *mb0 = nullptr,
-                       const double *mb1 = nullptr,
-                       double *smb = nullptr, int ndiag = 0, unsigned *sig = nullptr, int sig_tile = 0,
-                       double *xmb = nullptr);
+int launch_panel_pair(double *A, size_t lda, int c0, int r0, int r1, const double *q0, const double *q1, unsigned *out0,
+                      unsigned *xr, unsigned *out1, unsigned *abort_word, hipStream_t s, const double *mb0 = nullptr,
+                      const double *mb1 = nullptr,
+                      double *smb = nullptr, int ndiag = 0, unsigned *sig = nullptr, int sig_tile = 0,
+                      double *xmb = nullptr,
+                      unsigned *done = nullptr);
 constexpr size_t PANEL_XMBOX_DOUBLES = 8 * 4 * 256;
 constexpr size_t PANEL_SMBOX_DOUBLES = 4 * 16 * 4 * 256;
 void launch_update(double *A, size_t lda, int k0, int K, int ti0, int ti1, int tj0, int tj1,
@@ -124,7 +125,8 @@
                    int band_hi = -1, int ext0 = 0,
                    int skew = 0,
                    int trim64 = 0,
-                   int skip_lo = 0, int skip_hi = 0);
+                   int skip_lo = 0, int skip_hi = 0,
+                   unsigned *near = nullptr, int near_lo = 0);
 void set_update_waves(int nw);
 void set_update_w8_max_tiles(int ntiles);
 void set_update_c_wt(int on);
@@ -133,7 +135,7 @@
                         int group, int world, int rank, unsigned *sig = nullptr, int sig_tile = -1,
                         unsigned *wait_word = nullptr, unsigned *abort_word = nullptr, unsigned *queue = nullptr,
                         int band_hi = -1, int ext0 = 0, int skew = 0, int kblk = 0, int trim64 = 0,
-                        const int *pmap = nullptr, int skip_lo = 0, int skip_hi = 0);
+                        const int *pmap = nullptr, int skip_lo = 0, int skip_hi = 0, unsigned *near = nullptr, int near_lo = 0);
 void launch_pack_rows(const double *A, size_t lda, int col0, int ncols, double *dst, size_t ldp, const int *pmap, int ti_lo,
                       int ti_hi, long long slot_lo, long long slot_hi, hipStream_t s);
 
```

After: 121.0 (median of 6 runs). About the same (+0.2%).
